# yonkshi/SPAIR_pytorch

Hardware: AMD Instinct MI355X
Metric: SPAIR train images/sec + ELBO, 128x128 scattered-MNIST, batch 256 (higher is better)
Workload: dtype bf16

## Files before the change

### include/spair_hip.h

```cpp
#pragma once
#include <stddef.h>
#include <stdint.h>
#ifdef __cplusplus
extern "C" {
#endif

#define SPAIR_DTYPE_F32 0
#define SPAIR_DTYPE_BF16 1

typedef struct SpairDims {
    int B, C, I, G;
    int P, A, F, NP;
    int n_conv;
    int conv_k[8], conv_s[8], conv_c[8];
    int pad_pre, pad_post, cell_px;
    int dtype;
    int align_corners;
    float anchor;
    float max_yx, min_yx, max_hw, min_hw;
    float obj_logit_scale, alpha_logit_scale, alpha_logit_bias;
    float vae_beta;
    float prior_mean[6], prior_std[6];
    int obj_conv, oc_n;
    int oc_k[4], oc_s[4], oc_c[4];
    int lookback;
    int Iw, Gw, pad_post_w;
} SpairDims;

#define SPAIR_ABI_VERSION 3
int spair_abi_version(void);

typedef struct SpairStep {
    float wheel;
    float count_prior_prob;
    float kl_scale;
    int train;
    int flags;
    int draw_noise;
    unsigned long long noise_seed;
    int* status;
    int* status_host;
} SpairStep;

int spair_init(void);

int spair_param_count(const SpairDims* d);
int spair_param_info(const SpairDims* d, int idx, char* name, int name_cap, int64_t* offset, int64_t* shape4, int* ndim);
int64_t spair_param_total(const SpairDims* d);
int64_t spair_workspace_bytes(const SpairDims* d);

typedef struct SpairStepIO {
    const float* params;
    const float* x;
    float* eps_box;
    float* eps_attr;
    float* eps_depth;
    float* u_pres;
    void* workspace;
    float* loss_out;
    float* recon;
    float* z_where;
    float* z_pres;
    float* inv_den;
    const float* grad_loss;
    float* grads;
    void* ev_decoder;
    void* ev_cells;
    void* ev_backbone;
    const float* grad_recon;
    const float* grad_z_where;
    const float* grad_z_pres;
    float* aux_scratch;
    float* grad_x;
    void* x_scratch;
    int bce_target;
} SpairStepIO;
int spair_forward(const SpairDims* d, const SpairStep* st, const SpairStepIO* io, void* stream);
int spair_backward(const SpairDims* d, const SpairStep* st, const SpairStepIO* io, void* stream);
int spair_grad_buckets(const SpairDims* d, int64_t* lo3, int64_t* hi3);
int64_t spair_input_grad_scratch_bytes(const SpairDims* d);
int spair_adam(float* params, const float* grads, float* exp_avg, float* exp_avg_sq, int64_t n, float lr,
               float beta1, float beta2, float eps, int step, void* stream);
int spair_adam_guarded(float* params, const float* grads, float* exp_avg, float* exp_avg_sq, int64_t n, float lr,
                       float beta1, float beta2, float eps, int step, const int* skip, int* counters, void* stream);
int spair_host_word_alloc(int** out);
int spair_host_word_free(int* word);
int spair_export_map(const SpairDims* d, const void* workspace, int which, float* out, void* stream);
int spair_chain_stamps(const SpairDims* d, const void* workspace, unsigned long long* out, int n, void* stream);
int spair_chain_stamp_layout(int* fwd_per_wavefront, int* fwd_glimpse_interval, int* bwd_per_wavefront);
#define SPAIR_STEP_PLAN_INTS 38
#define SPAIR_RENDER_MMA 0
#define SPAIR_RENDER_GEN2 1
#define SPAIR_RENDER_GEN1 2
#define SPAIR_RENDER_COLOUR 3
#define SPAIR_CONV_GEMM 0
#define SPAIR_CONV_PATCH 1
#define SPAIR_CONV_PER_CLASS 2
#define SPAIR_CONV_PW_STACK 3
#define SPAIR_STEM_PATCH 0
#define SPAIR_STEM_GEMM 1
#define SPAIR_STEM_WGRAD16 2
#define SPAIR_STEM_GENERIC 3
int spair_step_plan(const SpairDims* d, const void* workspace, int flags, int input_grad, int* out, int n);
int spair_workspace_view(const SpairDims* d, const void* workspace, int flags, int input_grad, const char* name, long long* out);
int spair_workspace_view_name(const SpairDims* d, int idx, char* name, int name_cap);
int spair_chain_stamp_wavefronts(const SpairDims* d);
int spair_chain_sync_status(const SpairDims* d, const void* workspace, int* out, void* stream);
int spair_noise_fill(const SpairDims* d, uint64_t seed, float* eps_box, float* eps_attr, float* eps_depth, float* u_pres, void* stream);

int spair_prof_enable(int enable);
int spair_prof_select(unsigned long long slot_mask);
int spair_prof_read(float* ms, int* counts, int nslots);

int spair_gemm_nt(const float* A, int lda, const void* B, int ldb, float* C, int ldc, int M, int N, int K,
                  const float* bias, const float* relu_mask, int ldmask, int relu, int accumulate, int dtype,
                  void* stream);
int spair_gemm_tn(const float* A, int lda, const float* B, int ldb, float* C, int ldc, int M, int N, int R,
                  int dtype, void* stream);
int spair_gemm_nt_conv(const float* In, const int* conv13, const void* B, int ldb, float* C, int ldc, int M,
                       int N, int K, const float* bias, const float* relu_mask, int ldmask, int relu,
                       int accumulate, const int* cmap8, int dtype, void* stream);
int spair_gemm_tn_conv(const float* A, int lda, const float* In, const int* conv13, float* C, int ldc, int M,
                       int N, int R, int dtype, void* stream);
int spair_colsum(const float* A, int lda, int R, int N, float* out, void* stream);
int spair_objconv_gather(int transposed, const float* in, const long long* in6, const float* W, const float* bias, float* out,
                         const long long* out6, const float* gate, int k, int s, int relu, long long R, void* stream);
int spair_objconv_wgrad(const float* small, const long long* small6, const float* big, const long long* big6, float* G,
                        float* bias_small, int k, int s, long long R, void* stream);
int spair_gemm_nt16(const void* A, int lda, const void* B, int ldb, void* C, int ldc, int M, int N, int K,
                    const float* bias, const void* relu_mask, int ldmask, int mask_bf16, int relu, int c_bf16,
                    const int* conv13, const int* cmap8, void* stream);
int spair_gemm_tn16(const void* A, int lda, const void* B, int ldb, int b_bf16, float* C, int ldc, int M, int N,
                    int R, const int* conv13, int cw_cin, int cw_taps, float* colsum_out, float* scratch,
                    long long scratch_floats, void* stream);
int spair_stem_wgrad16(const void* dY, const float* xpad, float* dW, float* db, float* scratch,
                       long long scratch_floats, int B, int Hin, int stride, int Hout, void* stream);
int spair_conv1x1_stack_fwd16(const void* X, const void* const* W, const int* ldw, const int* cout,
                              const float* const* bias, void* const* Y, float* Ylast, int ldlast, int M, int L,
                              void* stream);
int spair_conv1x1_stack_bwd16(const void* dY, int ldd, int kd, const void* const* Wd, const int* ldw, const int* cout,
                              const void* const* gate, void* const* dX, int M, int L, void* stream);
int spair_metrics(const float* z_where, const float* z_pres, const float* bbox, const float* count, int B, int G,
                  int image_side, int K, float* scratch, float* out, void* stream);
int spair_batch_jaccard(const float* box_a, const float* box_b, int B, int A, int Bn, float* iou, void* stream);
int spair_scenes_generate(uint64_t seed, long long first, int B, int I, int K, int size_min, int size_max, float* image,
                          float* bbox, long long* count, float* scratch, void* stream);
int spair_cast_bf16(const float* src, int ld_src, void* dst, int ld_dst, long long rows, int cols, void* stream);
int spair_stn_glimpse_fwd(const float* x, const float* nbox, int B, float* glimpse, int ld_gl, int R, int C,
                          int I, int P, int align_corners, void* stream);
int spair_stn_glimpse_bwd(const float* x, const float* nbox, int B, const float* dglimpse, int ld_gl,
                          float* dnbox, int R, int C, int I, int P, int align_corners, void* stream);
int spair_input_grad_glimpse(const float* nbox, int B, int ncell, const float* dglimpse, int ld_gl, float* out, int C, int I, int P,
                             int align_corners, void* stream);
int spair_input_grad_stem(const void* dact0, int dact_bf16, const float* w, int B, int C, int I, int pad_pre, int k, int s, int Hout,
                          int Cout, const float* add, float* grad_x, void* stream);
int spair_stn_inverse_fwd(const float* sprites, const float* nbox, float* out, int N, int C, int P, int I, int align_corners,
                          void* stream);
int spair_stn_inverse_bwd(const float* sprites, const float* nbox, const float* grad_out, float* dsprites, float* dnbox, int N,
                          int C, int P, int I, int align_corners, void* stream);
int spair_render_fwd(const float* sprites, int ld_s, const float* nbox, const float* pres, const float* depth,
                     const float* x, float* recon, float* aux , float* bce_partial,
                     int B, int HW, int C, int I, int P, int align_corners, void* stream);
int spair_render_bwd(const float* sprites, int ld_s, const float* nbox, const float* pres, const float* depth,
                     const float* aux, const float* grad_loss, float* dlogits, float* dnbox, float* dpres, float* ddepth,
                     int B, int HW, int C, int I, int P, int align_corners, float obj_scale, float alpha_scale, void* stream);
int spair_render_fwd_rgb(const float* sprites, int ld_s, const float* nbox, const float* pres, const float* depth, const float* x,
                         float* recon, float* aux, float* bce_partial, int B, int HW, int C, int I, int P, int align_corners, void* stream);
int spair_render_bwd_rgb(const float* sprites, int ld_s, const float* nbox, const float* pres, const float* depth, const float* aux,
                         const float* grad_loss, float* dlogits, float* dnbox, float* dpres, float* ddepth, int B, int HW, int C, int I,
                         int P, int align_corners, float obj_scale, float alpha_scale, void* stream);
int spair_stem_conv_fwd(const float* x, const float* w, const float* bias, void* out, int B, int I, int pad_pre, int Hin, int Hout,
                        int Cout, int stride, int out_bf16, void* stream);
int spair_conv_s2k4_fwd16(const void* in16, const void* wf16, const float* bias, void* out16, int B, int Hin, int Hout, void* stream);
int spair_conv_s2k4_dgrad16(const void* dout16, const void* wd0, const void* wd1, const void* wd2, const void* wd3, const void* gate16,
                            void* out16, int B, int Ho, void* stream);
int spair_stem_conv_fwd_mask(const float* x, const float* w, const float* bias, void* out, void* mask8, int B, int I, int pad_pre, int Hin,
                             int Hout, void* stream);
int spair_conv_s2k4_dgrad16_bits(const void* dout16, const void* wd0, const void* wd1, const void* wd2, const void* wd3,
                                 const void* gate_bits8, void* out16, int B, int Ho, void* stream);
int64_t spair_decoder_fwd16_scratch_bytes(int n_out);
int spair_decoder_fwd16(const void* z_attr16, int ld_za, const float* W0, const float* b0, const float* W1, const float* b1,
                        const float* W2, const float* b2, void* H1, void* H2, void* sprites, int ld_s, long long N, int A, int n_out,
                        float obj_scale, float alpha_scale, float alpha_bias, void* stream_buf, void* stream);
int spair_decoder_bwd16(const void* dlogits16, int ld_s, const void* W2t16, int ld2, const void* W1t16, const void* W0t16, const void* H2,
                        const void* H1, void* dH2, void* dH1, float* d_z_attr, int ld_dza, long long N, int A, int n_out, void* stream);
int spair_render_fwd16(const void* sprites_f16, int ld_s, const float* nbox, const float* pres, const float* depth,
                       const float* x, float* recon, float* aux, float* bce_partial, int B, int HW, int C, int I, int P,
                       int align_corners, void* stream);
int spair_render_bwd16(const void* sprites_f16, int ld_s, const float* nbox, const float* pres, const float* depth,
                       const float* aux, const float* grad_loss, void* dlogits_bf16, float* dnbox, float* dpres, float* ddepth,
                       int B, int HW, int C, int I, int P, int align_corners, float obj_scale, float alpha_scale, void* stream);
int spair_render_prep(const float* nbox, const float* pres, const float* depth, void* records, int B, int HW, int I, int P,
                      int align_corners, void* stream);
int spair_render_fwd16m(const void* sprites_f16, int ld_s, const void* records, const float* x, float* recon, float* aux,
                        float* bce_partial, int B, int HW, int C, int I, int P, int align_corners, void* stream);
int spair_render_bwd16r(const void* sprites_f16, int ld_s, const float* nbox, const float* pres, const float* depth, const void* records,
                        const float* aux, const float* grad_loss, void* dlogits_bf16, float* dnbox, float* dpres, float* ddepth,
                        int B, int HW, int C, int I, int P, int align_corners, float obj_scale, float alpha_scale, void* stream);
int spair_render_owner(const void* sprites, int ld_s, int s16, int ch, const float* nbox, const float* pres, const float* depth,
                       const int* cidx, float threshold, int* owner, float* owner_weight, float* coverage, int* area, int B, int HW, int I,
                       int Iw, int P, int align_corners, void* stream);
int spair_parse_owner(const SpairDims* d, const void* workspace, int flags, float threshold, int* owner, float* owner_weight,
                      float* coverage, int* area, void* stream);
int spair_cell_rows(const SpairDims* d, const void* workspace, int* out, void* stream);
#ifdef __cplusplus
}
#endif
```

### spair_pytorch_amd/_lib.py

```python
import ctypes
import os

import torch

_HERE = os.path.dirname(os.path.abspath(__file__))
LIB_PATH = os.environ.get("SPAIR_HIP_LIB") or os.path.join(_HERE, "libspair_hip.so")

_ERR = {-1: "bad shape", -2: "unsupported dtype", -3: "kernel launch failed", -4: "unsupported configuration",
        -5: "misaligned leading dimension / size"}

_lib = None
ABI_VERSION = 3


class SpairHipError(RuntimeError):
    pass


class SpairDims(ctypes.Structure):
    _fields_ = [("B", ctypes.c_int), ("C", ctypes.c_int), ("I", ctypes.c_int), ("G", ctypes.c_int),
                ("P", ctypes.c_int), ("A", ctypes.c_int), ("F", ctypes.c_int), ("NP", ctypes.c_int),
                ("n_conv", ctypes.c_int), ("conv_k", ctypes.c_int * 8), ("conv_s", ctypes.c_int * 8),
                ("conv_c", ctypes.c_int * 8), ("pad_pre", ctypes.c_int), ("pad_post", ctypes.c_int),
                ("cell_px", ctypes.c_int), ("dtype", ctypes.c_int), ("align_corners", ctypes.c_int),
                ("anchor", ctypes.c_float), ("max_yx", ctypes.c_float), ("min_yx", ctypes.c_float),
                ("max_hw", ctypes.c_float), ("min_hw", ctypes.c_float), ("obj_logit_scale", ctypes.c_float),
                ("alpha_logit_scale", ctypes.c_float), ("alpha_logit_bias", ctypes.c_float),
                ("vae_beta", ctypes.c_float), ("prior_mean", ctypes.c_float * 6), ("prior_std", ctypes.c_float * 6),
                ("obj_conv", ctypes.c_int), ("oc_n", ctypes.c_int), ("oc_k", ctypes.c_int * 4), ("oc_s", ctypes.c_int * 4),
                ("oc_c", ctypes.c_int * 4), ("lookback", ctypes.c_int),
                ("Iw", ctypes.c_int), ("Gw", ctypes.c_int), ("pad_post_w", ctypes.c_int)]


class SpairStep(ctypes.Structure):
    _fields_ = [("wheel", ctypes.c_float), ("count_prior_prob", ctypes.c_float), ("kl_scale", ctypes.c_float),
                ("train", ctypes.c_int), ("flags", ctypes.c_int), ("draw_noise", ctypes.c_int), ("noise_seed", ctypes.c_uint64),
                ("status", ctypes.c_void_p), ("status_host", ctypes.c_void_p)]


class SpairStepIO(ctypes.Structure):
    _fields_ = [(n, ctypes.c_void_p) for n in (
        "params", "x", "eps_box", "eps_attr", "eps_depth", "u_pres", "workspace",
        "loss_out", "recon", "z_where", "z_pres", "inv_den",
        "grad_loss", "grads", "ev_decoder", "ev_cells", "ev_backbone",
        "grad_recon", "grad_z_where", "grad_z_pres", "aux_scratch", "grad_x", "x_scratch")] + [("bce_target", ctypes.c_int)]


_STEP_ARGS = [ctypes.POINTER(SpairDims), ctypes.POINTER(SpairStep), ctypes.POINTER(SpairStepIO), ctypes.c_void_p]


def lib():
    global _lib
    if _lib is None:
        if not os.path.exists(LIB_PATH):
            raise SpairHipError(
                "libspair_hip.so is not built (%s). Run `python -c 'import __graft_entry__ as g; g.build()'` "
                "or `python -m spair_pytorch_amd._build`. There is no CPU/PyTorch fallback." % LIB_PATH)
        h = ctypes.CDLL(LIB_PATH)
        got = h.spair_abi_version() if hasattr(h, "spair_abi_version") else None
        if got != ABI_VERSION:
            raise SpairHipError("%s has ABI version %s, this package needs %d: rebuild it (python -m spair_pytorch_amd._build)"
                                % (LIB_PATH, got, ABI_VERSION))
        for f, args in ((h.spair_forward, _STEP_ARGS), (h.spair_backward, _STEP_ARGS),
                        (h.spair_step_plan, [ctypes.POINTER(SpairDims), ctypes.c_void_p, ctypes.c_int, ctypes.c_int,
                                             ctypes.POINTER(ctypes.c_int), ctypes.c_int])):
            f.argtypes, f.restype = args, ctypes.c_int
        _declare_parse(h)
        _lib = h
    return _lib


def _declare_parse(h):
    vp, i, f = ctypes.c_void_p, ctypes.c_int, ctypes.c_float
    h.spair_render_owner.argtypes = [vp, i, i, i, vp, vp, vp, vp, f, vp, vp, vp, vp, i, i, i, i, i, i, vp]
    h.spair_parse_owner.argtypes = [ctypes.POINTER(SpairDims), vp, i, f, vp, vp, vp, vp, vp]
    h.spair_cell_rows.argtypes = [ctypes.POINTER(SpairDims), vp, vp, vp]
    for fn in (h.spair_render_owner, h.spair_parse_owner, h.spair_cell_rows):
        fn.restype = i


def check(rc, what):
    if rc != 0:
        raise SpairHipError("%s failed: %s (code %d)" % (what, _ERR.get(rc, "unknown"), rc))


def ptr(t):
    if t is None:
        return ctypes.c_void_p(0)
    return ctypes.c_void_p(t.data_ptr())


def stream():
    return ctypes.c_void_p(torch.cuda.current_stream().cuda_stream)


RENDER_FAMILIES = ("MMA", "GEN2", "GEN1", "COLOUR")


def step_plan(dims, workspace, flags=0):
    out = (ctypes.c_int * 8)()
    check(lib().spair_step_plan(ctypes.byref(dims), int(workspace), int(flags), 0, out, 8), "spair_step_plan")
    return dict(fwd=RENDER_FAMILIES[out[0]], bwd=RENDER_FAMILIES[out[1]], rec=bool(out[2]), s16=bool(out[3]), g16=bool(out[4]),
                chain=bool(out[5]), dec_fused=bool(out[6]))


CONV_KERNELS = ("GEMM", "PATCH", "PER_CLASS", "PW_STACK")
STEM_WGRADS = ("PATCH", "GEMM", "WGRAD16", "GENERIC")
STEP_PLAN_INTS = 38


def step_plan_n(dims, workspace, flags=0, input_grad=False):
    out = (ctypes.c_int * STEP_PLAN_INTS)()
    check(lib().spair_step_plan(ctypes.byref(dims), int(workspace), int(flags), int(bool(input_grad)), out, STEP_PLAN_INTS),
          "spair_step_plan")
    layers = range(dims.n_conv)
    return dict(side=bool(out[8]), dec_dgrad_fused=bool(out[9]), dec_wgrad_grouped=bool(out[10]), dec_wgrad_late=bool(out[11]), pw0=out[12],
                stem=STEM_WGRADS[out[13]], fwd=tuple(CONV_KERNELS[out[14 + i]] for i in layers),
                dgrad=tuple(CONV_KERNELS[out[22 + i]] for i in layers), gate_bits=tuple(bool(out[30 + i]) for i in layers))


VIEW_DTYPES = (torch.float32, torch.bfloat16, torch.float16)


def workspace_view_names(dims):
    f, buf, names = lib().spair_workspace_view_name, ctypes.create_string_buffer(128), []
    while f(ctypes.byref(dims), len(names), buf, 128) == 0:
        names.append(buf.value.decode())
    return names


def workspace_view(dims, workspace, name, flags=0, input_grad=False):
    out = (ctypes.c_longlong * 6)()
    check(lib().spair_workspace_view(ctypes.byref(dims), ctypes.c_void_p(int(workspace)), int(flags), int(bool(input_grad)),
                                     name.encode(), out), "spair_workspace_view(%s)" % name)
    return dict(offset=out[0], rows=out[1], cols=out[2], ld=out[3], dtype=VIEW_DTYPES[out[4]], written=bool(out[5]))


def render_owner(sprites, channels, nbox, pres, depth, B, HW, I, Iw, P, align_corners=False, threshold=0.5, cell_rows=None):
    if sprites.dtype not in (torch.float16, torch.float32) or sprites.stride(1) != 1:
        raise SpairHipError("sprites must be fp16 or fp32 rows")
    dev = sprites.device
    owner = torch.empty(B, I, Iw, device=dev, dtype=torch.int32)
    weight, cover = (torch.empty(B, I, Iw, device=dev, dtype=torch.float32) for _ in range(2))
    area = torch.empty(B, HW, device=dev, dtype=torch.int32)
    nbox, pres, depth = (t.contiguous().float() for t in (nbox, pres, depth))
    rows = None if cell_rows is None else cell_rows.to(device=dev, dtype=torch.int32).contiguous()
    if sprites.shape[0] != B * HW or nbox.numel() != 4 * B * HW or pres.numel() != B * HW or depth.numel() != B * HW or \
            (rows is not None and rows.numel() != HW):
        raise SpairHipError("render_owner: operands do not have B * HW rows")
    check(lib().spair_render_owner(ptr(sprites), int(sprites.stride(0)), int(sprites.dtype == torch.float16), int(channels), ptr(nbox),
                                   ptr(pres), ptr(depth), ptr(rows), float(threshold), ptr(owner), ptr(weight), ptr(cover), ptr(area),
                                   int(B), int(HW), int(I), int(Iw), int(P), int(bool(align_corners)), stream()), "spair_render_owner")
    return owner, weight, cover, area
```

### spair_pytorch_amd/csrc/backbone.h

```cpp
#pragma once
#include "common.h"
#include "spair_hip.h"

bool conv_s2k4_patch_fwd16_supported(int B, int Hin, int Hout, int cin, int cout, int k, int s_);
int conv_s2k4_patch_fwd16(const void* in, const void* wf, const float* bias, void* out, int B, int Hin, int Hout, int cin, int cout, int k, int s_,
                          hipStream_t s, void* mask = nullptr);
bool conv_s2k4_patch_dgrad16_supported(int B, int Ho, int hin, int cin, int cout, int k, int s_);
bool conv_s2k4_patch_dgrad16_stem_supported(int B, int Ho, int hin, int cin, int cout, int k, int s_, int stem_hin, int stem_s, long long stem_part_cap);
int conv_s2k4_patch_dgrad16(const void* dout, const void* const* wd, const void* gate, void* out, int B, int Ho, int hin, int cin, int cout, int k,
                            int s_, const float* stem_xp, int stem_hin, int stem_s, float* stem_part, long long stem_part_cap, float* stem_dw,
                            float* stem_db, hipStream_t s, const void* gate_bits = nullptr);

enum ConvKernel { CONV_GEMM = SPAIR_CONV_GEMM, CONV_PATCH = SPAIR_CONV_PATCH, CONV_PER_CLASS = SPAIR_CONV_PER_CLASS, CONV_PW_STACK = SPAIR_CONV_PW_STACK };
enum StemWgrad { STEM_PATCH = SPAIR_STEM_PATCH, STEM_GEMM = SPAIR_STEM_GEMM, STEM_WGRAD16 = SPAIR_STEM_WGRAD16, STEM_GENERIC = SPAIR_STEM_GENERIC };
```

### spair_pytorch_amd/csrc/chain.hip

```cpp
#include <type_traits>
#include "cell_math.h"
#include "chain.h"
#include "stn_math.h"

namespace {

constexpr int MT = 16;
constexpr int F = 100, REC = 56, CTX = 224, A_ = 50, NP = 100, GLN = 784, PG = 28;
constexpr int CH_PAD = 16;
constexpr int KC = 352, LD_XC = KC + CH_PAD;
constexpr int KX = 160, LD_XT = KX + CH_PAD;
constexpr int KG = 800, LD_GL = KG + CH_PAD;
constexpr int LD_H = 256 + CH_PAD;
constexpr int LD_O = 112;
static_assert(CHAIN_PACK[CW_BOX0].ksplit == F + CTX && CHAIN_PACK[CW_BOX0].kpad0 == KC && CHAIN_PACK[CW_BOX0].KT * 32 == KC, "box0 pack");
static_assert(CHAIN_PACK[CW_Z0].ksplit == F + CTX && CHAIN_PACK[CW_Z0].kpad0 == KC && CHAIN_PACK[CW_Z0].KT * 32 == KC + KX, "z0 pack");
static_assert(CHAIN_PACK[CW_OBJ0].ksplit == F + CTX && CHAIN_PACK[CW_OBJ0].kpad0 == KC && CHAIN_PACK[CW_OBJ0].KT * 32 == KC + KX, "obj0 pack");
static_assert(CHAIN_PACK[CW_ENC0].ksplit == GLN && CHAIN_PACK[CW_ENC0].kpad0 == KG && CHAIN_PACK[CW_ENC0].KT * 32 == KG, "enc0 pack");

__device__ __forceinline__ void lds_barrier() {
    asm volatile("s_waitcnt lgkmcnt(0)" ::: "memory");
    __builtin_amdgcn_s_barrier();
    asm volatile("" ::: "memory");
}
// ... 58 lines not shown
__device__ __forceinline__ float ch_log(float x) { return 0.693147180559945f * __builtin_amdgcn_logf(x); }

template <int PIECES, int PB>
__device__ __forceinline__ void copy_rows8(const void* lds_, int lds_pitch, void* hbm_, unsigned hbm_pitch, const int* row_r, int r0, int nc, int lane) {
    constexpr int NI = (PIECES + 7) / 8;
    typedef unsigned int uv __attribute__((ext_vector_type(PB / 4)));
    const int row = r0 + (lane >> 3), p0 = lane & 7;
    const char* src = reinterpret_cast<const char*>(lds_) + row * lds_pitch + p0 * PB;
    char* dst = reinterpret_cast<char*>(hbm_) + ((unsigned)row_r[row] * hbm_pitch + (unsigned)(p0 * PB));
    uv v[NI];
#pragma unroll
    for (int i = 0; i < NI; ++i)
        if (8 * (i + 1) <= PIECES || p0 + 8 * i < PIECES) v[i] = *reinterpret_cast<const uv*>(src + i * 8 * PB);
    if (row < nc) {
#pragma unroll
        for (int i = 0; i < NI; ++i)
            if (8 * (i + 1) <= PIECES || p0 + 8 * i < PIECES) CH_GSTORE(reinterpret_cast<uv*>(dst + i * 8 * PB), v[i]);
    }
}
template <int PIECES, int PB>
__device__ __forceinline__ void copy_rows_w(const void* lds, int lds_pitch, void* hbm, size_t hbm_pitch, const int* row_r, int nc, int lane) {
    copy_rows8<PIECES, PB>(lds, lds_pitch, hbm, (unsigned)hbm_pitch, row_r, 0, nc, lane);
    if (nc > 8) copy_rows8<PIECES, PB>(lds, lds_pitch, hbm, (unsigned)hbm_pitch, row_r, 8, nc, lane);
}

template <int KT0, int KT1, int NT, int NT0 = 0>
__device__ __forceinline__ void wg_gemm_t(const __bf16* inA, int ldA, const __bf16* inB, int ldB, const uint4* __restrict__ Wp, WPipe& p,
                                          const float* bias_l, f32x4& acc, int wave, int lane) {
    constexpr int KT = KT0 + KT1;
    static_assert(KT <= 16, "all activation fragments of the stage are held in registers");
    const uint4* base = tile_base<KT, NT, NT0>(Wp, wave, lane);
    const int nt = min(NT0 + wave, NT - 1);
    const __bf16* pa = inA + (lane & 15) * ldA + (lane >> 4) * 8;
    const __bf16* pb = (KT1 > 0) ? inB + (lane & 15) * ldB + (lane >> 4) * 8 : pa;
    bf16x8 x[KT];
#pragma unroll
    for (int kt = 0; kt < KT; ++kt)
        x[kt] = *reinterpret_cast<const bf16x8*>((kt < KT0) ? pa + kt * 32 : pb + (kt - KT0) * 32);
    acc = *reinterpret_cast<const f32x4*>(bias_l + nt * 16 + (lane >> 4) * 4);
    __builtin_amdgcn_sched_barrier(0);
#pragma unroll
    for (int f = 0; f < KT; ++f) {
        acc = __builtin_amdgcn_mfma_f32_16x16x32_bf16(as_frag(p.q[f % RD]), x[f], acc, 0, 0, 0);
        if (f + RD < KT) p.q[f % RD] = base[(size_t)(f + RD) * 64];
    }
}

template <int KTOT, int KSKIP, int NT>
__device__ __forceinline__ void pipe_fill_k(const uint4* __restrict__ Wp, WPipe& p, int wave, int lane) {
    const uint4* base = tile_base<KTOT, NT, 0>(Wp, wave, lane) + (size_t)KSKIP * 64;
#pragma unroll
    for (int f = 0; f < KTOT - KSKIP; ++f) p.q[f] = base[f * 64];
}
template <int KTOT, int KSKIP>
__device__ __forceinline__ void wg_gemm_tk(const __bf16* inB, int ldB, WPipe& p, f32x4& acc, int lane) {
    constexpr int KT = KTOT - KSKIP;
    static_assert(KT <= RD, "the remaining fragments sit in the ring");
    const __bf16* pb = inB + (lane & 15) * ldB + (lane >> 4) * 8;
    bf16x8 x[KT];
#pragma unroll
    for (int kt = 0; kt < KT; ++kt) x[kt] = *reinterpret_cast<const bf16x8*>(pb + kt * 32);
    __builtin_amdgcn_sched_barrier(0);
#pragma unroll
    for (int f = 0; f < KT; ++f) acc = __builtin_amdgcn_mfma_f32_16x16x32_bf16(as_frag(p.q[f]), x[f], acc, 0, 0, 0);
}
template <int KTOT, int NT, int K0, int N>
__device__ __forceinline__ void early_fill(const uint4* __restrict__ Wa, const uint4* __restrict__ Wb, WPipe& p, int wave, int lane) {
    static_assert(2 * N <= RD, "two fragments per k-step");
    const uint4* ba = tile_base<KTOT, NT, 0>(Wa, wave, lane) + (size_t)K0 * 64;
    const uint4* bb = tile_base<KTOT, NT, 0>(Wb, wave, lane) + (size_t)K0 * 64;
#pragma unroll
    for (int j = 0; j < N; ++j) { p.q[2 * j] = ba[j * 64]; p.q[2 * j + 1] = bb[j * 64]; }
}
template <int N>
__device__ __forceinline__ void early_mfma(const bf16x8 (&x)[N], const WPipe& p, f32x4& accA, f32x4& accB) {
#pragma unroll
    for (int j = 0; j < N; ++j) {
        accA = __builtin_amdgcn_mfma_f32_16x16x32_bf16(as_frag(p.q[2 * j]), x[j], accA, 0, 0, 0);
        accB = __builtin_amdgcn_mfma_f32_16x16x32_bf16(as_frag(p.q[2 * j + 1]), x[j], accB, 0, 0, 0);
    }
}
__device__ __forceinline__ void buf_store8_nt(__amdgpu_buffer_rsrc_t r, unsigned byte_off, unsigned lo, unsigned hi) {
    __builtin_amdgcn_raw_buffer_store_b64(u32x2_t{lo, hi}, r, (int)byte_off, 0, 2);
}
__device__ __forceinline__ void buf_store16_nt(__amdgpu_buffer_rsrc_t r, unsigned byte_off, u32x4_t v) {
    __builtin_amdgcn_raw_buffer_store_b128(v, r, (int)byte_off, 0, 2);
}

template <int KT>
__device__ __forceinline__ void pipe_fill2(const uint4* __restrict__ Wp, WPipe& p, int wave, int lane) {
    const uint4* b0 = Wp + (size_t)wave * KT * 64 + lane;
    const uint4* b1 = Wp + (size_t)(wave + 8) * KT * 64 + lane;
#pragma unroll
    for (int s = 0; s < RD; ++s) p.q[s] = ((s & 1) ? b1 : b0)[(s >> 1) * 64];
}
template <int KT, int CH, int NRES>
__device__ __forceinline__ void wg_gemm_t2(const __bf16* in, int ld, const uint4* __restrict__ Wp, WPipe& p, const uint4 (&res)[2 * NRES + 1],
                                           const float* bias_l, f32x4& acc0, f32x4& acc1, int wave, int lane) {
    static_assert(KT % CH == 0 && RD % 2 == 0, "whole chunks; ring slots alternate between the two tiles");
    constexpr int NCH = KT / CH, AH = RD / 2;
    constexpr int KS = KT - NRES;
    const uint4* b0 = Wp + (size_t)wave * KT * 64 + lane;
    const uint4* b1 = Wp + (size_t)(wave + 8) * KT * 64 + lane;
    const __bf16* pa = in + (lane & 15) * ld + (lane >> 4) * 8;
    bf16x8 x[2][CH];
#pragma unroll
    for (int j = 0; j < CH; ++j) x[0][j] = *reinterpret_cast<const bf16x8*>(pa + j * 32);
    acc0 = *reinterpret_cast<const f32x4*>(bias_l + wave * 16 + (lane >> 4) * 4);
    acc1 = *reinterpret_cast<const f32x4*>(bias_l + (wave + 8) * 16 + (lane >> 4) * 4);
#pragma unroll
    for (int c = 0; c < NCH; ++c) {
        if (c + 1 < NCH) {
#pragma unroll
            for (int j = 0; j < CH; ++j) x[(c + 1) & 1][j] = *reinterpret_cast<const bf16x8*>(pa + ((c + 1) * CH + j) * 32);
        }
        __builtin_amdgcn_sched_barrier(0);
#pragma unroll
        for (int j = 0; j < CH; ++j) {
            const int f = c * CH + j;
            if (f < KS) {
                acc0 = __builtin_amdgcn_mfma_f32_16x16x32_bf16(as_frag(p.q[(2 * f) % RD]), x[c & 1][j], acc0, 0, 0, 0);
                if (f + AH < KS) p.q[(2 * f) % RD] = b0[(size_t)(f + AH) * 64];
                acc1 = __builtin_amdgcn_mfma_f32_16x16x32_bf16(as_frag(p.q[(2 * f + 1) % RD]), x[c & 1][j], acc1, 0, 0, 0);
                if (f + AH < KS) p.q[(2 * f + 1) % RD] = b1[(size_t)(f + AH) * 64];
            } else {
                acc0 = __builtin_amdgcn_mfma_f32_16x16x32_bf16(as_frag(res[2 * (f - KS)]), x[c & 1][j], acc0, 0, 0, 0);
                acc1 = __builtin_amdgcn_mfma_f32_16x16x32_bf16(as_frag(res[2 * (f - KS) + 1]), x[c & 1][j], acc1, 0, 0, 0);
            }
        }
    }
}

template <int KT, int NT>
__device__ __forceinline__ void pipe_fill_s(const uint4* __restrict__ Whi, const uint4* __restrict__ Wlo, WPipe& p, int wave, int lane) {
    const size_t o = (size_t)min(wave, NT - 1) * KT * 64 + lane;
#pragma unroll
    for (int s_ = 0; s_ < RD; ++s_)
        if ((s_ >> 1) < KT) p.q[s_] = ((s_ & 1) ? Wlo : Whi)[o + (s_ >> 1) * 64];
}
template <int KT, int NT, int CH>
__device__ __forceinline__ void wg_gemm_s(const __bf16* inHi, const __bf16* inLo, int ld, const uint4* __restrict__ Whi, const uint4* __restrict__ Wlo,
                                          WPipe& p, const float* bias_l, f32x4& acc, int wave, int lane) {
    constexpr int NCH = (KT + CH - 1) / CH, AH = RD / 2;
    const int nt = min(wave, NT - 1);
    const size_t o = (size_t)nt * KT * 64 + lane;
    const int eoff = (lane & 15) * ld + (lane >> 4) * 8;
    bf16x8 xh[2][CH], xl[2][CH];
#pragma unroll
    for (int j = 0; j < CH; ++j)
        if (j < KT) { xh[0][j] = *reinterpret_cast<const bf16x8*>(inHi + eoff + j * 32); xl[0][j] = *reinterpret_cast<const bf16x8*>(inLo + eoff + j * 32); }
    acc = *reinterpret_cast<const f32x4*>(bias_l + nt * 16 + (lane >> 4) * 4);
#pragma unroll
    for (int c = 0; c < NCH; ++c) {
        if (c + 1 < NCH) {
#pragma unroll
            for (int j = 0; j < CH; ++j)
                if ((c + 1) * CH + j < KT) {
                    xh[(c + 1) & 1][j] = *reinterpret_cast<const bf16x8*>(inHi + eoff + ((c + 1) * CH + j) * 32);
                    xl[(c + 1) & 1][j] = *reinterpret_cast<const bf16x8*>(inLo + eoff + ((c + 1) * CH + j) * 32);
                }
        }
        __builtin_amdgcn_sched_barrier(0);
#pragma unroll
        for (int j = 0; j < CH; ++j) {
            const int f = c * CH + j;
            if (f < KT) {
                const bf16x8 wh = as_frag(p.q[(2 * f) % RD]), wl = as_frag(p.q[(2 * f + 1) % RD]);
                acc = __builtin_amdgcn_mfma_f32_16x16x32_bf16(wl, xh[c & 1][j], acc, 0, 0, 0);
                acc = __builtin_amdgcn_mfma_f32_16x16x32_bf16(wh, xl[c & 1][j], acc, 0, 0, 0);
// ... 1226 lines not shown
```

### spair_pytorch_amd/csrc/common.h

```cpp
#pragma once
#include <hip/hip_runtime.h>
#include <stdint.h>
#include <atomic>

#define SPAIR_OK 0
#define SPAIR_ERR_SHAPE (-1)
#define SPAIR_ERR_DTYPE (-2)
#define SPAIR_ERR_LAUNCH (-3)
#define SPAIR_ERR_UNSUPPORTED (-4)
#define SPAIR_ERR_ALIGN (-5)

#define SPAIR_F32 0
#define SPAIR_BF16 1

#define SPAIR_CHECK_LAUNCH()                                   \
    do {                                                       \
        hipError_t e__ = hipGetLastError();                    \
        if (e__ != hipSuccess) return SPAIR_ERR_LAUNCH;        \
    } while (0)


static inline int spair_dyn_lds_once(const void* fn, int bytes, std::atomic<unsigned long long>& done) {
    int dev = 0;
    if (hipGetDevice(&dev) != hipSuccess) return SPAIR_ERR_LAUNCH;
// ... 6 lines not shown
}
static inline int spair_num_cus() {
    static std::atomic<int> cus[64];
    int dev = 0;
    if (hipGetDevice(&dev) != hipSuccess) return 256;
    int n = cus[dev & 63].load(std::memory_order_relaxed);
    if (n <= 0) {
        if (hipDeviceGetAttribute(&n, hipDeviceAttributeMultiprocessorCount, dev) != hipSuccess || n <= 0) n = 256;
        cus[dev & 63].store(n, std::memory_order_relaxed);
    }
    return n;
}

typedef float f32x4 __attribute__((ext_vector_type(4)));
typedef __bf16 bf16x8 __attribute__((ext_vector_type(8)));
typedef __bf16 bf16x4 __attribute__((ext_vector_type(4)));
typedef unsigned short u16;

static inline int ceil_div(int a, int b) { return (a + b - 1) / b; }
static inline int round_up(int a, int b) { return ceil_div(a, b) * b; }

struct ConvDesc {
    int Hin, Win, Cin;
    int Hout, Wout;
    int kh, kw;
    int sy, sx;
    int dky, dkx;
    int oy, ox;
};

struct RowMap {
    int Hout, Wout;
    int Hc, Wc;
    int osy, osx, ooy, oox;
};

__device__ __forceinline__ float sigmoidf_(float x) { return 1.0f / (1.0f + expf(-x)); }

template <int CTRL>
__device__ __forceinline__ float dpp_add_(float v) {
    return v + __builtin_bit_cast(float, __builtin_amdgcn_update_dpp(0, __builtin_bit_cast(int, v), CTRL, 0xf, 0xf, true));
}
__device__ __forceinline__ float wave_reduce_sum(float v) {
    v = dpp_add_<0xB1>(v);
    v = dpp_add_<0x4E>(v);
    v = dpp_add_<0x141>(v);
    v = dpp_add_<0x140>(v);
    const int i = __builtin_bit_cast(int, v);
    return (__builtin_bit_cast(float, __builtin_amdgcn_readlane(i, 0)) + __builtin_bit_cast(float, __builtin_amdgcn_readlane(i, 16))) +
           (__builtin_bit_cast(float, __builtin_amdgcn_readlane(i, 32)) + __builtin_bit_cast(float, __builtin_amdgcn_readlane(i, 48)));
}

#if defined(__HIPCC__)
__device__ __forceinline__ void wave_lds_fence() {
    __builtin_amdgcn_fence(__ATOMIC_RELEASE, "wavefront");
    __builtin_amdgcn_wave_barrier();
    __builtin_amdgcn_fence(__ATOMIC_ACQUIRE, "wavefront");
}
typedef unsigned int u32x4_t __attribute__((ext_vector_type(4)));
#define BUF_OOB 0xfffffff0u
__device__ __forceinline__ __amdgpu_buffer_rsrc_t buf_rsrc(const void* p) {
    const unsigned long long a = reinterpret_cast<unsigned long long>(p);
    const unsigned lo = __builtin_amdgcn_readfirstlane((unsigned)a), hi = __builtin_amdgcn_readfirstlane((unsigned)(a >> 32));
    void* q = reinterpret_cast<void*>(((unsigned long long)hi << 32) | lo);
    return __builtin_amdgcn_make_buffer_rsrc(q, (short)0, (int)0xffffff00u, 0x00020000);
}
__device__ __forceinline__ uint4 buf_load16(__amdgpu_buffer_rsrc_t r, unsigned byte_off) {
    const u32x4_t v = __builtin_amdgcn_raw_buffer_load_b128(r, (int)byte_off, 0, 0);
    return make_uint4(v.x, v.y, v.z, v.w);
}
typedef unsigned int u32x2_t __attribute__((ext_vector_type(2)));
__device__ __forceinline__ void buf_store2(__amdgpu_buffer_rsrc_t r, unsigned byte_off, unsigned short bits) {
    __builtin_amdgcn_raw_buffer_store_b16((short)bits, r, (int)byte_off, 0, 0);
}
__device__ __forceinline__ void buf_store4(__amdgpu_buffer_rsrc_t r, unsigned byte_off, unsigned bits) {
    __builtin_amdgcn_raw_buffer_store_b32((int)bits, r, (int)byte_off, 0, 0);
}
__device__ __forceinline__ void buf_store8(__amdgpu_buffer_rsrc_t r, unsigned byte_off, unsigned lo, unsigned hi) {
    __builtin_amdgcn_raw_buffer_store_b64(u32x2_t{lo, hi}, r, (int)byte_off, 0, 0);
}
__device__ __forceinline__ void buf_store16(__amdgpu_buffer_rsrc_t r, unsigned byte_off, uint4 v) {
    __builtin_amdgcn_raw_buffer_store_b128(u32x4_t{v.x, v.y, v.z, v.w}, r, (int)byte_off, 0, 0);
}
#endif

__device__ __forceinline__ float block_reduce_sum_256(float v, float* smem4) {
    v = wave_reduce_sum(v);
    const int w = threadIdx.x >> 6;
    __syncthreads();
    if ((threadIdx.x & 63) == 0) smem4[w] = v;
    __syncthreads();
    return smem4[0] + smem4[1] + smem4[2] + smem4[3];
}
```

### spair_pytorch_amd/csrc/conv_s2.hip

```cpp
#include <numeric>
#include "common.h"
#include "backbone.h"

namespace {

constexpr int CP_BM = 256, CP_C = 128;
constexpr int CP_PPX = 392;
constexpr int CP_PATCH_B = CP_PPX * 128;
constexpr int CP_BT_B = 128 * 128;
constexpr int CP_NPIECE_W = 5;
constexpr int CP_LDS = 3 * CP_BT_B + 2 * CP_PATCH_B + 1024;
constexpr int CP_LDC = CP_C + 16;

struct ConvPatchArgs {
    const u16* in; const u16* wf; const float* bias; u16* out;
    unsigned char* mask;
    int B, Hin, Hout, M, K;
    int tpi;
};

template <int W>
__device__ __forceinline__ void cp_wait() { asm volatile("s_waitcnt vmcnt(%0)" ::"n"(W) : "memory"); }

__global__ __launch_bounds__(768, 3) void k_conv_s2k4_patch(ConvPatchArgs a) {
    extern __shared__ __attribute__((aligned(16))) char cp_sm[];
    char* bt = cp_sm;
    char* patch = cp_sm + 3 * CP_BT_B;
    const int tid = threadIdx.x, lane = tid & 63, wave = __builtin_amdgcn_readfirstlane(tid >> 6);
    const int q = lane >> 4, r16 = lane & 15;
    const int Hout = a.Hout, Ws = Hout + 1, Hs = Hout + 1;
    int m0, mend;
    if (a.tpi) {
        const int img = blockIdx.x / a.tpi, HH = Hout * Hout;
        m0 = img * HH + (blockIdx.x - img * a.tpi) * CP_BM;
        mend = min(m0 + CP_BM, (img + 1) * HH);
    } else {
        m0 = blockIdx.x * CP_BM;
        mend = min(m0 + CP_BM, a.M);
    }
    const int mlast = mend - 1;
    const int g0 = m0 / Hout, g1 = mlast / Hout;
    const int L0 = (g0 + g0 / Hout) * Ws + (m0 - g0 * Hout);
    const int npx = (g1 + g1 / Hout + 1) * Ws + (mlast - g1 * Hout) + 1 - L0 + 1;

    const bool loader = wave >= 8;
    const int lw = wave & 3;
    const int wm = (wave >> 1) & 3, wn = wave & 1;
    const __amdgpu_buffer_rsrc_t rin = buf_rsrc(a.in), rwf = buf_rsrc(a.wf);
    auto glds = [&](__amdgpu_buffer_rsrc_t rs, unsigned byte_off, char* dst) {
        __builtin_amdgcn_raw_ptr_buffer_load_lds(rs, (__attribute__((address_space(3))) void*)dst, 16, (int)byte_off, 0, 0, 0);
    };
    auto issue_b = [&](int kt) {
        const bool live = kt < (a.K >> 6);
        char* dst = bt + (kt % 3) * CP_BT_B;
#pragma unroll
        for (int p = 0; p < 4; ++p) {
            const int piece = lw * 4 + p, n = piece * 8 + (lane >> 3), pos = lane & 7, c = pos ^ (n & 7);
            glds(rwf, live ? ((unsigned)n * (unsigned)a.K + (unsigned)kt * 64u + (unsigned)c * 8u) * 2u : BUF_OOB, dst + piece * 1024);
        }
    };
    auto issue_patch = [&](int st, int part) {
        const int cls = st >> 1, half = st & 1, py = cls >> 1, px = cls & 1;
        char* dst = patch + (st & 1) * CP_PATCH_B;
#pragma unroll
        for (int e = 0; e < CP_NPIECE_W; ++e) {
            const int piece = (part * 4 + lw) * CP_NPIECE_W + e;
            const int pp = piece * 8 + (lane >> 3), pos = lane & 7, c = pos ^ (pp & 7);
            const int pg = L0 + pp, E = pg / Ws, xx = pg - E * Ws;
            const int b = E / Hs, yy = E - b * Hs;
            const bool ok = st < 8 && pp < npx && b < a.B;
            const unsigned off = (((unsigned)(b * a.Hin + 2 * yy + py) * (unsigned)a.Hin + (unsigned)(2 * xx + px)) * CP_C + half * 64 + c * 8) * 2u;
            glds(rin, ok ? off : BUF_OOB, piece < CP_PPX / 8 ? dst + piece * 1024 : cp_sm + 3 * CP_BT_B + 2 * CP_PATCH_B);
        }
    };

    f32x4 acc[4][4];
#pragma unroll
    for (int i = 0; i < 4; ++i)
#pragma unroll
        for (int j = 0; j < 4; ++j) acc[i][j] = (f32x4){0.f, 0.f, 0.f, 0.f};

    if (loader) {
#pragma unroll
        for (int part = 0; part < 3; ++part) issue_patch(0, part);
        issue_b(0);
        issue_b(1);
        cp_wait<4>();
        for (int st = 0; st < 8; ++st) {
#pragma unroll
            for (int j4 = 0; j4 < 4; ++j4) {
                const int kt = st * 4 + j4;
                __builtin_amdgcn_s_barrier();
                asm volatile("" ::: "memory");
                if (j4 != 3) issue_patch(st + 1, j4);
                issue_b(kt + 2);
                if (j4 == 3) cp_wait<4>(); else cp_wait<4 + CP_NPIECE_W>();
            }
        }
        __builtin_amdgcn_s_barrier();
    } else {
        int pbase[4];
#pragma unroll
        for (int i = 0; i < 4; ++i) {
            const int m = min(m0 + wm * 64 + i * 16 + r16, mlast);
            const int g = m / Hout, x = m - g * Hout;
            pbase[i] = (g + g / Hout) * Ws + x - L0;
        }
        for (int st = 0; st < 8; ++st) {
            const char* pb = patch + (st & 1) * CP_PATCH_B;
#pragma unroll
            for (int j4 = 0; j4 < 4; ++j4) {
                const int kt = st * 4 + j4;
                __builtin_amdgcn_s_barrier();
                asm volatile("" ::: "memory");
                const char* bs = bt + (kt % 3) * CP_BT_B;
                const int tap = (j4 >> 1) * Ws + (j4 & 1);
#pragma unroll
                for (int ks = 0; ks < 2; ++ks) {
                    bf16x8 af[4], bfr[4];
                    const int c = ks * 4 + q;
#pragma unroll
                    for (int i = 0; i < 4; ++i) {
                        const int pp = pbase[i] + tap;
                        af[i] = *reinterpret_cast<const bf16x8*>(pb + pp * 128 + ((c ^ (pp & 7)) << 4));
                    }
#pragma unroll
                    for (int j = 0; j < 4; ++j) {
                        const int n = wn * 64 + j * 16 + r16;
                        bfr[j] = *reinterpret_cast<const bf16x8*>(bs + n * 128 + ((c ^ (n & 7)) << 4));
                    }
#pragma unroll
                    for (int i = 0; i < 4; ++i)
#pragma unroll
                        for (int j = 0; j < 4; ++j) acc[i][j] = __builtin_amdgcn_mfma_f32_16x16x32_bf16(af[i], bfr[j], acc[i][j], 0, 0, 0);
                }
            }
        }
        __builtin_amdgcn_s_barrier();
    }
    asm volatile("s_waitcnt vmcnt(0)" ::: "memory");
    __syncthreads();

    __bf16* cs = reinterpret_cast<__bf16*>(patch);
    if (!loader) {
#pragma unroll
        for (int j = 0; j < 4; ++j) {
            const int n = wn * 64 + j * 16 + r16;
            const float bv = a.bias[n];
#pragma unroll
            for (int i = 0; i < 4; ++i)
#pragma unroll
                for (int r = 0; r < 4; ++r) cs[(wm * 64 + i * 16 + q * 4 + r) * CP_LDC + n] = (__bf16)fmaxf(acc[i][j][r] + bv, 0.f);
        }
    }
    __syncthreads();
    const __amdgpu_buffer_rsrc_t rout = buf_rsrc(a.out);
    if (tid < 512) {
#pragma unroll
        for (int it = 0; it < CP_BM / 32; ++it) {
            const int row = it * 32 + (tid >> 4), ch = (tid & 15) * 8;
            const uint4 v = *reinterpret_cast<const uint4*>(cs + row * CP_LDC + ch);
            buf_store16(rout, (m0 + row) < mend ? ((unsigned)(m0 + row) * CP_C + ch) * 2u : BUF_OOB, v);
            if (a.mask) {
                auto nz2 = [](unsigned w) { return (unsigned)((int)(w << 16) > 0) | ((unsigned)((int)w >> 16 > 0) << 1); };
                const unsigned byte = nz2(v.x) | (nz2(v.y) << 2) | (nz2(v.z) << 4) | (nz2(v.w) << 6);
                if ((m0 + row) < mend) a.mask[(size_t)(m0 + row) * 16 + (tid & 15)] = (unsigned char)byte;
            }
        }
    }
}

}

static int cp_plan(int B, int Hin, int Hout, int cin, int cout, int k, int s_, int& tiles_out, int& tpi_out) {
    if (cin != CP_C || cout != CP_C || k != 4 || s_ != 2 || Hin != 2 * Hout + 2 || B <= 0 || Hout <= 0) return SPAIR_ERR_UNSUPPORTED;
    const long long M = (long long)B * Hout * Hout;
    if (M * CP_C >= (1ll << 31) || (long long)B * Hin * Hin * CP_C >= (1ll << 31)) return SPAIR_ERR_UNSUPPORTED;
    auto window = [&](long long m0, long long ml) {
        const long long g0 = m0 / Hout, g1 = ml / Hout;
        return (int)((g1 + g1 / Hout + 1) * (Hout + 1) + (ml - g1 * Hout) + 1 - ((g0 + g0 / Hout) * (Hout + 1) + (m0 - g0 * Hout)) + 1);
    };
    int tiles = (int)((M + CP_BM - 1) / CP_BM), tpi = 0, worst = 0;
    const long long period = (long long)Hout * Hout / std::gcd((long long)CP_BM, (long long)Hout * Hout);
    const bool walk = std::min<long long>(tiles, period) <= 65536;
    for (int t = 0; walk && t < tiles && t < period; ++t)
        worst = std::max(worst, window((long long)t * CP_BM, std::min<long long>((long long)(t + 1) * CP_BM, M) - 1));
    if (walk && tiles > period) worst = std::max(worst, window((long long)(tiles - 1) * CP_BM, M - 1));
    if (!walk || worst > CP_PPX) {
        const int HH = Hout * Hout;
        tpi = (HH + CP_BM - 1) / CP_BM;
        worst = 0;
        for (int t = 0; t < tpi; ++t) worst = std::max(worst, window((long long)t * CP_BM, std::min<long long>((long long)(t + 1) * CP_BM, HH) - 1));
        if (worst > CP_PPX) return SPAIR_ERR_UNSUPPORTED;
        tiles = B * tpi;
    }
    tiles_out = tiles; tpi_out = tpi;
    return SPAIR_OK;
}
bool conv_s2k4_patch_fwd16_supported(int B, int Hin, int Hout, int cin, int cout, int k, int s_) {
    int t, p;
    return cp_plan(B, Hin, Hout, cin, cout, k, s_, t, p) == SPAIR_OK;
}
int conv_s2k4_patch_fwd16(const void* in, const void* wf, const float* bias, void* out, int B, int Hin, int Hout, int cin, int cout, int k, int s_,
                          hipStream_t s, void* mask) {
    int tiles = 0, tpi = 0;
    { const int rc = cp_plan(B, Hin, Hout, cin, cout, k, s_, tiles, tpi); if (rc != SPAIR_OK) return rc; }
    const long long M = (long long)B * Hout * Hout;
    static std::atomic<unsigned long long> attr_done{0};
    if (spair_dyn_lds_once(reinterpret_cast<const void*>(&k_conv_s2k4_patch), CP_LDS, attr_done) != SPAIR_OK) return SPAIR_ERR_LAUNCH;
    ConvPatchArgs a;
    a.in = reinterpret_cast<const u16*>(in); a.wf = reinterpret_cast<const u16*>(wf); a.bias = bias; a.out = reinterpret_cast<u16*>(out);
    a.mask = reinterpret_cast<unsigned char*>(mask);
    a.B = B; a.Hin = Hin; a.Hout = Hout; a.M = (int)M; a.K = 16 * CP_C; a.tpi = tpi;
    hipLaunchKernelGGL(k_conv_s2k4_patch, dim3(tiles), dim3(768), CP_LDS, s, a);
    SPAIR_CHECK_LAUNCH();
    return SPAIR_OK;
}

extern "C" int spair_conv_s2k4_fwd16(const void* in16, const void* wf16, const float* bias, void* out16, int B, int Hin, int Hout, void* stream) {
    return conv_s2k4_patch_fwd16(in16, wf16, bias, out16, B, Hin, Hout, 128, 128, 4, 2, (hipStream_t)stream);
}
```

### spair_pytorch_amd/csrc/engine.hip

```cpp
#include <string.h>
#include <stdio.h>
#include <algorithm>
#include <mutex>
#include <vector>

#include "backbone.h"
#include "cells.h"
#include "gemm.h"
#include "misc.h"
#include "chain.h"
#include "dec_fused.h"
#include "objconv.h"
#include "render.h"

#define TRY(expr)                      \
    do {                               \
        int rc__ = (expr);             \
        if (rc__ != SPAIR_OK) return rc__; \
    } while (0)


#define SP_PROF_SLOTS 24
#define SP_PROF_POOL 8192
struct ProfState {
// ... 23 lines not shown
    int i; hipStream_t s;
    ProfScope(int slot, hipStream_t st) : i(prof_begin(slot, st)), s(st) {}
    ~ProfScope() { prof_end(i, s); }
};

extern "C" int spair_prof_enable(int enable) {
    std::lock_guard<std::mutex> lock(g_prof_mu);
    if (enable && g_prof.n_events == 0) {
        for (int i = 0; i < 2 * SP_PROF_POOL; ++i)
            if (hipEventCreate(&g_prof.ev[i]) != hipSuccess) return SPAIR_ERR_LAUNCH;
        g_prof.n_events = 2 * SP_PROF_POOL;
    }
    g_prof.enabled = enable ? 1 : 0;
    if (enable == 1) g_prof.used = 0;
    return SPAIR_OK;
}
extern "C" int spair_prof_select(unsigned long long mask) {
    std::lock_guard<std::mutex> lock(g_prof_mu);
    g_prof.mask = mask;
    return SPAIR_OK;
}
extern "C" int spair_prof_read(float* ms, int* counts, int nslots) {
    std::lock_guard<std::mutex> lock(g_prof_mu);
    for (int i = 0; i < g_prof.used; ++i) {
        float t = 0.f;
        if (hipEventSynchronize(g_prof.ev[2 * i + 1]) != hipSuccess) return SPAIR_ERR_LAUNCH;
        if (hipEventElapsedTime(&t, g_prof.ev[2 * i], g_prof.ev[2 * i + 1]) != hipSuccess) return SPAIR_ERR_LAUNCH;
        const int sl = g_prof.slot[i];
        if (sl >= 0 && sl < nslots) { ms[sl] += t; counts[sl] += 1; }
    }
    g_prof.used = 0;
    return SPAIR_OK;
}
enum { PS_PREP = 0, PS_BACKBONE_FWD, PS_CELLS_FWD, PS_DECODER_FWD, PS_COUNT_KL, PS_RENDER_FWD, PS_LOSS, PS_RENDER_BWD, PS_DECODER_BWD,
       PS_CELLS_BWD, PS_CELLS_WGRAD, PS_BACKBONE_BWD, PS_CONV1_FWD, PS_DEC2_FWD, PS_STN_FWD, PS_ADAM, PS_DEC2_WGRAD, PS_DEC2_DGRAD };

static int validate(const SpairDims& d) {
    if (d.B <= 0 || d.I <= 0 || d.G <= 0 || d.P <= 0 || d.A <= 0 || d.F <= 0 || d.NP <= 0) return SPAIR_ERR_SHAPE;
    if (d.Iw <= 0 || d.Gw <= 0 || d.pad_post_w < 0 || d.pad_post < 0 || d.pad_pre < 0) return SPAIR_ERR_SHAPE;
    if (d.C < 1 || d.C > 3) return SPAIR_ERR_UNSUPPORTED;
    if (d.C != 1 && d.obj_conv) return SPAIR_ERR_UNSUPPORTED;
    if (d.n_conv < 1 || d.n_conv > SP_MAX_CONV) return SPAIR_ERR_SHAPE;
    if (d.dtype != SPAIR_F32 && d.dtype != SPAIR_BF16) return SPAIR_ERR_DTYPE;
    if ((d.F & 3) || (d.NP & 3)) return SPAIR_ERR_ALIGN;
    int h = d.I + d.pad_pre + d.pad_post, wd = d.Iw + d.pad_pre + d.pad_post_w;
    for (int i = 0; i < d.n_conv; ++i) {
        if (d.conv_k[i] < 1 || d.conv_s[i] < 1 || (d.conv_c[i] & 7)) return SPAIR_ERR_SHAPE;
        if (i > 0 && d.conv_k[i] > 1 && (d.conv_k[i] % d.conv_s[i] != 0 || d.conv_s[i] > 2)) return SPAIR_ERR_UNSUPPORTED;
        if (i > 0 && d.conv_k[i] == 1 && d.conv_s[i] != 1) return SPAIR_ERR_UNSUPPORTED;
        h = (h - d.conv_k[i]) / d.conv_s[i] + 1;
        wd = (wd - d.conv_k[i]) / d.conv_s[i] + 1;
    }
    if (h != d.G || wd != d.Gw) return SPAIR_ERR_SHAPE;
    if ((long long)d.G * d.Gw + 1 > 1025) return SPAIR_ERR_UNSUPPORTED;
    if (d.A + 5 > 64) return SPAIR_ERR_UNSUPPORTED;
    if (d.lookback < 0 || d.lookback > 3) return SPAIR_ERR_UNSUPPORTED;
    if (d.lookback > 1 && std::max(d.G, d.Gw) > 32) return SPAIR_ERR_UNSUPPORTED;
    if (d.obj_conv) {
        if (d.oc_n < 1 || d.oc_n > 4) return SPAIR_ERR_SHAPE;
        int hh = d.P, ci = d.C;
        for (int i = 0; i < d.oc_n; ++i) {
            if (d.oc_k[i] < 1 || d.oc_s[i] < 1 || d.oc_c[i] < 1 || d.oc_k[i] > hh) return SPAIR_ERR_SHAPE;
            if ((long long)ci * d.oc_c[i] * d.oc_k[i] * d.oc_k[i] > 256 * 36 || d.oc_c[i] > 256) return SPAIR_ERR_UNSUPPORTED;
            const int ho = (hh - d.oc_k[i]) / d.oc_s[i] + 1;
            hh = ho; ci = d.oc_c[i];
        }
        if (((ci * hh * hh) & 7) || ((d.P * d.P * (d.C + 1)) & 7)) return SPAIR_ERR_ALIGN;
        if ((long long)(d.C + 1) * d.oc_c[0] * d.oc_k[0] * d.oc_k[0] > 256 * 36) return SPAIR_ERR_UNSUPPORTED;
    }
    return SPAIR_OK;
}

struct StepPlan {
    bool use_chain;
    bool use_dec_fused;
    RenderPlan rp;
    bool use_side;
    int pw0;
    ConvKernel conv_fwd[SP_MAX_CONV + 1], conv_dgrad[SP_MAX_CONV + 1];
    bool gate_bits[SP_MAX_CONV + 1];
    bool stem_bits;
    StemWgrad stem_wgrad;
    bool stem_unpadded;
    bool dec_dgrad_fused;
    bool dec_wgrad_grouped;
    bool dec_wgrad_late;
};

static RenderGeom render_geom(const SpairDims& d, const CellLayout& L, const CellBufs* b) {
    return {b ? b->nbox : nullptr, b ? b->rec + (L.REC - 1) : nullptr, b ? b->rec + (L.REC - 2) : nullptr, L.ld_rec, d.B, L.HW, d.I, d.P,
            d.align_corners, d.Iw};
}

static bool decoder_small_wgrad_grouped_supported(const ParamLayout& PL, const CellLayout& L) {
    const LinSpec &l1 = PL.lin[LIN_DEC1], &l0 = PL.lin[LIN_DEC0];
    return l1.in <= 128 && l0.in <= 128 && !(l1.out & 7) && !(l0.out & 7) && ceil_div(l1.out, 128) + ceil_div(l0.out, 128) <= SPAIR_TN_MAX_TILES &&
           std::min(round_up(l1.in, 8), SP_DEC_H1) >= l1.in && std::min(round_up(l0.in, 8), L.ld_rec) >= l0.in &&
           (long long)L.N * std::max(SP_DEC_H2, L.ld_rec) < (1ll << 31);
}

static StepPlan plan_step(const SpairDims& d, int flags, bool input_grad, const void* base) {
    const CellLayout L = make_cell_layout(d);
    const ParamLayout PL = make_param_layout(d);
    StepPlan p = {};
    const bool b16 = d.dtype == SPAIR_BF16;
    const bool square = spair_dims_square(d);
    const int per = d.P * d.P * (d.C + 1), ld_s = round_up(per, 8);
    p.use_chain = square && chain_fwd_supported(d) && !(flags & 1) && !d.obj_conv;
    const float* at = static_cast<const float*>(base);
    p.rp = render_plan(d, render_geom(d, L, nullptr), ld_s, at, at, at);
    p.use_dec_fused = p.rp.s16  && !(flags & 16) && PL.lin[LIN_DEC0].out == SP_DEC_H1 && PL.lin[LIN_DEC1].out == SP_DEC_H2 &&
                      dec_fused_supported(d.A, per, L.ld_rec, L.N, ld_s);
    p.use_side = !(flags & 4);
    const ConvSpec& c0 = PL.conv[0];
    const bool grey4 = square && c0.cin == 1 && c0.k == 4 && c0.cout == 128;
    const bool fuse_stem = b16 && grey4 && !(flags & 8) && !input_grad;
    const bool patch = square && b16 && !(flags & 32);
    p.stem_wgrad = b16 && grey4 ? STEM_WGRAD16 : STEM_GENERIC;
    p.stem_unpadded = square && misc_conv0_reads_unpadded(d.B, c0.hin, d.C, c0.k, c0.cout);
    p.stem_bits = square && misc_conv0_writes_mask(d.B, c0.hin, d.C, c0.k, c0.s, c0.cout, b16);
    const int n = PL.n_conv;
    p.pw0 = n;
    for (int i = n - 1; b16 && i >= 1; --i) {
        const ConvSpec& cs = PL.conv[i];
        if (cs.k != 1 || cs.s != 1 || cs.cin != 128 || (i == n - 1 ? cs.cout > 128 : cs.cout != 128) || n - i > 4 || PL.conv[i - 1].cout != 128) break;
        p.pw0 = i;
    }
    if (n - p.pw0 < 2) p.pw0 = n;
    bool bits = p.stem_bits;
    for (int i = 1; i < n; ++i) {
        const ConvSpec& cs = PL.conv[i];
        if (i >= p.pw0) { p.conv_fwd[i] = p.conv_dgrad[i] = CONV_PW_STACK; continue; }
        p.conv_fwd[i] = patch && conv_s2k4_patch_fwd16_supported(d.B, cs.hin, cs.hout, cs.cin, cs.cout, cs.k, cs.s) ? CONV_PATCH : CONV_GEMM;
        if (cs.k == 1) p.conv_dgrad[i] = CONV_GEMM;
        else if (patch && conv_s2k4_patch_dgrad16_supported(d.B, cs.hout, cs.hin, cs.cin, cs.cout, cs.k, cs.s)) {
            p.conv_dgrad[i] = CONV_PATCH;
            p.gate_bits[i] = bits;
            if (i == 1 && fuse_stem &&
                conv_s2k4_patch_dgrad16_stem_supported(d.B, cs.hout, cs.hin, cs.cin, cs.cout, cs.k, cs.s, c0.hin, c0.s, SPAIR_TN_PART_FLOATS))
                p.stem_wgrad = STEM_PATCH;
        } else if (b16 && cs.hin % cs.s == 0 && cs.win % cs.s == 0 && cs.s * cs.s <= 4) {
            p.conv_dgrad[i] = CONV_GEMM;
            const int M = d.B * ceil_div(cs.hin, cs.s) * ceil_div(cs.win, cs.s);
            if (i == 1 && fuse_stem && spair_nt16_stem_fusable(M, cs.cin, cs.s * cs.s, c0.hin, c0.s, SPAIR_TN_PART_FLOATS)) p.stem_wgrad = STEM_GEMM;
        } else p.conv_dgrad[i] = CONV_PER_CLASS;
        bits = p.conv_fwd[i] == CONV_PATCH;
    }
    const bool dec16 = b16 && !PL.oc_n;
    p.dec_dgrad_fused = dec16 && !(flags & 64) && dec_fused_bwd_supported(PL.lin[LIN_DEC0].in, per, L.N, ld_s, ld_s, L.ld_rec);
    p.dec_wgrad_grouped = dec16 && decoder_small_wgrad_grouped_supported(PL, L);
    p.dec_wgrad_late = dec16 && p.use_side && p.use_chain;
    return p;
}

struct Ws {
    int *cell_h, *cell_w, *cidx, *nbr, *cons, *diag_start;
    void* conv_wf[SP_MAX_CONV + 1];
    void* conv_wd[SP_MAX_CONV + 1][4];
    void* lin_wf[LIN_COUNT];
    void* lin_wt[LIN_COUNT];
    float *bias_boxh, *bias_zh;
    void* chain_w[CW_COUNT];
    void* chain_wlo[3];
    void* chain_wt[CW_COUNT];
    void* dec_stream;
    float* xpad;
    float *act[SP_MAX_CONV + 1], *dact[SP_MAX_CONV + 1];
    void* dLog16;
    unsigned char* act0_bits;
    unsigned char* act_bits[SP_MAX_CONV + 1];
    float *feat, *dfeat;
    CellBufs cb;
    float *Za, *Hd1, *Hd2, *S, *dLog, *dHd2, *dHd1;
    void *Za16, *dfeat16;
    float *tn_part, *tn_part2;
    float *aux, *bce_partial, *kl_partial, *klp, *gedge_part;
    void* rrec;
    float *oc_ea[4], *oc_dea[4];
    float *oc_dh, *oc_ddh;
    float *oc_da[4], *oc_dda[4];
    int* chain_sync;
    float *bnd_rec, *bnd_grad;
    unsigned long long* stamps;
    int ld_feat, ld_s;
    size_t total;
};

struct Carver {
    char* base;
    size_t off;
    template <class T> T* take(size_t n) {
        off = (off + 255) & ~(size_t)255;
        T* p = base ? reinterpret_cast<T*>(base + off) : nullptr;
        off += n * sizeof(T);
        return p;
    }
    void* take_bytes(size_t n) { return take<char>(n); }
};

static Ws carve(const SpairDims& d, void* base) {
    Ws w;
    memset(&w, 0, sizeof(w));
    const CellLayout L = make_cell_layout(d);
    const ParamLayout PL = make_param_layout(d);
    const StepPlan p = plan_step(d, 0, false, nullptr);
    Carver c{reinterpret_cast<char*>(base), 0};
    const size_t es = d.dtype == SPAIR_BF16 ? 2 : 4;
    const size_t N = (size_t)L.N;
    w.cell_h = c.take<int>(L.HW); w.cell_w = c.take<int>(L.HW); w.cidx = c.take<int>(L.HW);
    w.nbr = c.take<int>(L.NB * L.HW); w.cons = c.take<int>(L.NB * L.HW); w.diag_start = c.take<int>((L.LB + 1) * (L.G - 1) + L.Gw + 2);
    for (int i = 1; i < PL.n_conv; ++i) {
        const ConvSpec& cs = PL.conv[i];
        const size_t K = (size_t)cs.k * cs.k * cs.cin;
        w.conv_wf[i] = c.take_bytes((size_t)cs.cout * round_up((int)K, 8) * es);
        if (cs.k == 1) w.conv_wd[i][0] = c.take_bytes((size_t)cs.cin * round_up(cs.cout, 8) * es);
        else for (int q = 0; q < cs.s * cs.s; ++q) {
            const int T = cs.k / cs.s;
            w.conv_wd[i][q] = c.take_bytes((size_t)cs.cin * T * T * cs.cout * es);
        }
    }
    auto lin_alloc = [&](int id, int rows_total) {
        w.lin_wf[id] = c.take_bytes((size_t)rows_total * round_up(PL.lin[id].in, 8) * es);
        w.lin_wt[id] = c.take_bytes((size_t)PL.lin[id].in * round_up(rows_total, 8) * es);
    };
    for (int id = 0; id < LIN_COUNT; ++id) {
        if (id == LIN_BOXH0 || id == LIN_ZH0) continue;
        int rows = PL.lin[id].out;
        if (id == LIN_BOXH1) rows += PL.lin[LIN_BOXH0].out;
        if (id == LIN_ZH1) rows += PL.lin[LIN_ZH0].out;
        lin_alloc(id, rows);
// ... 221 lines not shown
    c.T = S * (G - 1) + Gw;
    c.dstart.assign(c.T + 1, 0);
    int n = 0;
    for (int t = 0; t < c.T; ++t) {
        c.dstart[t] = n;
        for (int h = 0; h < G; ++h) {
            const int w = t - S * h;
            if (w >= 0 && w < Gw) ++n;
        }
    }
    c.dstart[c.T] = n;
}

static int nt(Ctx& c, const float* A, int lda, const void* B, int ldb, float* C, int ldc, int M, int N, int K, const float* bias,
              const float* mask, int ldmask, int relu, const ConvDesc* conv = nullptr, const RowMap* cmap = nullptr) {
    GemmNT g;
    memset(&g, 0, sizeof(g));
    g.A = A; g.lda = lda; g.B = B; g.ldb = ldb; g.C = C; g.ldc = ldc; g.M = M; g.N = N; g.K = K;
    g.bias = bias; g.mask = mask; g.ldmask = ldmask; g.relu = relu;
    if (conv) g.conv = *conv;
    if (cmap) { g.cmap = *cmap; g.use_cmap = 1; }
    return spair_gemm_nt_impl(g, conv != nullptr, c.d.dtype, c.s);
}
static int tn(Ctx& c, const float* A, int lda, int M, const float* B, int ldb, int N, float* C, int ldc, int R, float* colsum = nullptr,
              const ConvDesc* conv = nullptr, int cw_cin = 0, int cw_taps = 0) {
    GemmTN g;
    memset(&g, 0, sizeof(g));
    g.A = A; g.lda = lda; g.B = B; g.ldb = ldb; g.C = C; g.ldc = ldc;
    g.M = round_up(M, 4); g.N = round_up(N, 4); g.Mstore = M; g.Nstore = N; g.R = R; g.colsum_out = colsum;
    g.cw_cin = cw_cin; g.cw_taps = cw_taps;
    if (conv) g.conv = *conv;
    return spair_gemm_tn_impl(g, conv != nullptr, c.d.dtype, c.s);
}
static bool conv_kperm(const Ctx& c, const ConvSpec& cs) {
    return c.d.dtype == SPAIR_BF16 && cs.k > 1 && cs.s > 1 && cs.k % cs.s == 0 && cs.cin % 64 == 0 && cs.k * cs.k * cs.cin / 64 <= 64;
}
static void fill_ktab(GemmNT& g, const ConvSpec& cs) {
    const int T = cs.k / cs.s, TT = T * T, nh = cs.cin / 64;
    g.n_ktab = cs.k * cs.k * nh;
    for (int blk = 0; blk < g.n_ktab; ++blk) {
        const int tq = blk % TT, rr = blk / TT, h = rr % nh, cls = rr / nh;
        const int ky = cls / cs.s + cs.s * (tq / T), kx = cls % cs.s + cs.s * (tq % T);
        g.ktab[blk] = ((unsigned)ky << 24) | ((unsigned)kx << 16) | (unsigned)(h * 64);
    }
}
static int nt16(Ctx& c, const void* A, int lda, const void* B, int ldb, void* C, int ldc, int c_bf16, int M, int N, int K, const float* bias,
                const void* mask, int ldmask, int relu, const ConvDesc* conv = nullptr, const RowMap* cmap = nullptr,
                const ConvSpec* fwd_cs = nullptr) {
    GemmNT g;
    memset(&g, 0, sizeof(g));
    g.A = reinterpret_cast<const float*>(A); g.lda = lda; g.B = B; g.ldb = ldb; g.C = reinterpret_cast<float*>(C); g.ldc = ldc; g.c_bf16 = c_bf16;
    g.M = M; g.N = N; g.K = K; g.bias = bias; g.mask = reinterpret_cast<const float*>(mask); g.ldmask = ldmask; g.mask_bf16 = 1; g.relu = relu;
    if (conv) g.conv = *conv;
    if (cmap) { g.cmap = *cmap; g.use_cmap = 1; }
    if (fwd_cs && conv_kperm(c, *fwd_cs)) fill_ktab(g, *fwd_cs);
    return spair_gemm_nt16_impl(g, conv != nullptr, c.s);
}
static int tn16(Ctx& c, const void* A, int lda, int M, const void* B, int ldb, int N, bool b_bf16, float* C, int ldc, int R, float* colsum,
                const ConvDesc* conv = nullptr, int cw_cin = 0, int cw_taps = 0) {
    GemmTN g;
    memset(&g, 0, sizeof(g));
    g.A = reinterpret_cast<const float*>(A); g.lda = lda; g.B = reinterpret_cast<const float*>(B); g.ldb = ldb; g.C = C; g.ldc = ldc;
    g.M = round_up(M, 8); g.N = round_up(N, b_bf16 ? 8 : 4); g.Mstore = M; g.Nstore = N; g.R = R; g.colsum_out = colsum;
    g.cw_cin = cw_cin; g.cw_taps = cw_taps;
    g.part = c.tn_part; g.part_cap = SPAIR_TN_PART_FLOATS;
    if (conv) g.conv = *conv;
    return spair_gemm_tn16_impl(g, conv != nullptr, b_bf16, c.s);
}
static const void* bptr(const void* base, size_t elem_off, int dtype) {
    return reinterpret_cast<const char*>(base) + elem_off * (dtype == SPAIR_BF16 ? 2 : 4);
}

static int prep_weights(Ctx& c, bool need_dgrad, int part) {
    std::vector<PrepEntry> es;
    const int bf = c.d.dtype == SPAIR_BF16;
    auto push = [&](const float* src, void* dst, int rows, int cols, int ld, int mode, int bf16, int cin = 0, int cout = 0, int k = 0,
                    int py = 0, int px = 0, int T = 0, int s = 0) {
        PrepEntry e;
        memset(&e, 0, sizeof(e));
        e.src = src; e.dst = dst; e.rows = rows; e.cols = cols; e.ld = ld; e.mode = mode; e.bf16 = bf16;
        e.cin = cin; e.cout = cout; e.k = k; e.py = py; e.px = px; e.T = T; e.s = s;
        es.push_back(e);
    };
    for (int i = 1; part == 0 && i < c.PL.n_conv; ++i) {
        const ConvSpec& cs = c.PL.conv[i];
        const float* w = c.params + cs.w;
        const int K = cs.k * cs.k * cs.cin;
        if (cs.k == 1) {
            push(w, c.w.conv_wf[i], cs.cout, cs.cin, round_up(K, 8), 0, bf);
            if (need_dgrad) push(w, c.w.conv_wd[i][0], cs.cin, cs.cout, round_up(cs.cout, 8), 1, bf);
        } else {
            const bool perm = conv_kperm(c, cs);
            push(w, c.w.conv_wf[i], cs.cout, K, round_up(K, 8), 2, bf, cs.cin, cs.cout, cs.k, 0, 0, perm ? cs.k / cs.s : 0, perm ? cs.s : 0);
            if (need_dgrad) {
                const int T = cs.k / cs.s;
                for (int py = 0; py < cs.s; ++py)
                    for (int px = 0; px < cs.s; ++px)
                        push(w, c.w.conv_wd[i][py * cs.s + px], cs.cin, T * T * cs.cout, T * T * cs.cout, 3, bf, cs.cin, cs.cout, cs.k, py, px, T, cs.s);
            }
        }
    }
    for (int id = 0; part == 1 && id < LIN_COUNT; ++id) {
        if (id == LIN_BOXH0 || id == LIN_ZH0) continue;
        const LinSpec& l = c.PL.lin[id];
        if (!l.in || !l.out) continue;
        const int ldf = round_up(l.in, 8);
        int head0 = -1;
        if (id == LIN_BOXH1) head0 = LIN_BOXH0;
        if (id == LIN_ZH1) head0 = LIN_ZH0;
        const int rows_total = l.out + (head0 >= 0 ? c.PL.lin[head0].out : 0);
        const int ldt = round_up(rows_total, 8);
        push(c.params + l.w, c.w.lin_wf[id], l.out, l.in, ldf, 0, bf);
        if (need_dgrad) push(c.params + l.w, c.w.lin_wt[id], l.in, l.out, ldt, 1, bf);
        if (head0 >= 0) {
            const LinSpec& h = c.PL.lin[head0];
            push(c.params + h.w, const_cast<void*>(bptr(c.w.lin_wf[id], (size_t)l.out * ldf, c.d.dtype)), h.out, h.in, ldf, 0, bf);
            if (need_dgrad) push(c.params + h.w, const_cast<void*>(bptr(c.w.lin_wt[id], (size_t)l.out, c.d.dtype)), h.in, h.out, ldt, 1, bf);
        }
    }
    if (part == 1 && c.use_chain) {
        auto pack = [&](void* const* dst, int cw, int mode, int bf16) {
            const ChainPack& k = CHAIN_PACK[cw];
            for (int head = 0; head < (k.lin_head >= 0 ? 2 : 1); ++head) {
                const LinSpec& l = c.PL.lin[head ? k.lin_head : k.lin];
                PrepEntry e;
                memset(&e, 0, sizeof(e));
                e.src = c.params + l.w; e.dst = dst[cw]; e.rows = l.out; e.cols = l.in; e.mode = mode; e.bf16 = bf16;
                e.KT = mode == 4 ? k.KT : k.KTt; e.n_off = head ? c.L.NP : 0;
                if (mode == 4) { e.ksplit = k.ksplit; e.kpad0 = k.kpad0; }
                es.push_back(e);
            }
        };
        for (int cw = 0; cw < 3; ++cw) pack(c.w.chain_wlo, cw, 4, 2);
        for (int cw = 0; cw < CW_COUNT; ++cw) pack(c.w.chain_w, cw, 4, 1);
        for (int cw = 0; need_dgrad && cw < CW_COUNT; ++cw)
            if (CHAIN_PACK[cw].ntt) pack(c.w.chain_wt, cw, 5, 1);
    }
    if (part == 1 && c.use_dec_fused)
        TRY(dec_fused_pack(c.params + c.PL.lin[LIN_DEC0].w, c.params + c.PL.lin[LIN_DEC1].w, c.params + c.PL.lin[LIN_DEC2].w, c.d.A,
                           c.d.P * c.d.P * (c.d.C + 1), c.d.obj_logit_scale, c.d.alpha_logit_scale, c.w.dec_stream, c.s));
    if (part == 1) {
        push(c.params + c.PL.lin[LIN_BOXH1].b, c.w.bias_boxh, 1, c.L.NP, c.L.NP + 8, 0, 0);
        push(c.params + c.PL.lin[LIN_BOXH0].b, c.w.bias_boxh + c.L.NP, 1, 8, 8, 0, 0);
        push(c.params + c.PL.lin[LIN_ZH1].b, c.w.bias_zh, 1, c.L.NP, c.L.NP + 8, 0, 0);
        push(c.params + c.PL.lin[LIN_ZH0].b, c.w.bias_zh + c.L.NP, 1, 2, 8, 0, 0);
    }
    for (size_t i = 0; i < es.size(); i += SP_MAX_PREP) {
        PrepTable T;
        T.n = (int)std::min((size_t)SP_MAX_PREP, es.size() - i);
        for (int j = 0; j < T.n; ++j) T.e[j] = es[i + j];
        TRY(misc_prep(T, c.s));
    }
    return SPAIR_OK;
}

static ConvDesc fwd_desc(const ConvSpec& cs) {
    ConvDesc cd;
    cd.Hin = cs.hin; cd.Win = cs.win; cd.Cin = cs.cin; cd.Hout = cs.hout; cd.Wout = cs.wout; cd.kh = cs.k; cd.kw = cs.k;
    cd.sy = cs.s; cd.sx = cs.s; cd.dky = 1; cd.dkx = 1; cd.oy = 0; cd.ox = 0;
    return cd;
}

static int dgrad_class(const ConvSpec& cs, int py, int px, ConvDesc& dd, RowMap& rm) {
    const int T = cs.k / cs.s;
    const int Hc = (cs.hin - py + cs.s - 1) / cs.s, Wc = (cs.win - px + cs.s - 1) / cs.s;
    dd.Hin = cs.hout; dd.Win = cs.wout; dd.Cin = cs.cout; dd.Hout = Hc; dd.Wout = Wc; dd.kh = T; dd.kw = T;
    dd.sy = 1; dd.sx = 1; dd.dky = -1; dd.dkx = -1; dd.oy = 0; dd.ox = 0;
    rm.Hout = Hc; rm.Wout = Wc; rm.Hc = cs.hin; rm.Wc = cs.win; rm.osy = cs.s; rm.osx = cs.s; rm.ooy = py; rm.oox = px;
    return Hc > 0 && Wc > 0 ? Hc * Wc : 0;
}
static GemmNT dgrad_classes16(const Ctx& c, int i) {
    const ConvSpec &cs = c.PL.conv[i], &c0 = c.PL.conv[0];
    const int T = cs.k / cs.s;
    GemmNT g;
    memset(&g, 0, sizeof(g));
    g.M = c.d.B * dgrad_class(cs, 0, 0, g.conv, g.cmap); g.use_cmap = 1; g.N = cs.cin; g.K = T * T * cs.cout;
    g.ldb = g.K; g.C = c.w.dact[i - 1]; g.ldc = cs.cin; g.c_bf16 = 1; g.mask = c.w.act[i - 1]; g.ldmask = cs.cin; g.mask_bf16 = 1;
    g.nz = cs.s * cs.s;
    for (int q = 0; q < g.nz; ++q) g.Bz[q] = c.w.conv_wd[i][q];
    g.B = g.Bz[0];
    if (i == 1) { g.stem_xp = c.w.xpad; g.stem_hin = c0.hin; g.stem_s = c0.s; g.stem_part = c.w.tn_part; g.stem_part_cap = SPAIR_TN_PART_FLOATS; }
    return g;
}

static int make_ctx(Ctx& c, const SpairDims* d, const SpairStep* st, const SpairStepIO* io, void* stream, bool input_grad = false) {
    if (!d || !st || !io || !io->params || !io->x || !io->eps_box || !io->eps_attr || !io->eps_depth || !io->u_pres || !io->workspace)
        return SPAIR_ERR_SHAPE;
    c.d = spair_dims_norm(*d); c.st = *st;
    TRY(validate(c.d));
    d = &c.d;
    c.L = make_cell_layout(*d);
    c.PL = make_param_layout(*d);
    c.w = carve(*d, io->workspace);
    c.params = io->params; c.x = io->x; c.s = (hipStream_t)stream; c.tn_part = c.w.tn_part;
    CellHyper& H = c.H;
    H.wheel = st->wheel; H.kl_scale = st->kl_scale * d->vae_beta; H.img = (float)d->I; H.anchor = d->anchor;
    H.cell_over_img = (float)((double)d->cell_px / (double)d->I);
    H.img_w = (float)d->Iw;
    H.cell_over_w = (float)((double)d->cell_px / (double)d->Iw);
    H.max_yx = d->max_yx; H.min_yx = d->min_yx; H.max_hw = d->max_hw; H.min_hw = d->min_hw;
    H.range_yx = d->max_yx - d->min_yx; H.range_hw = d->max_hw - d->min_hw;
    for (int i = 0; i < 6; ++i) { H.prior_mean[i] = d->prior_mean[i]; H.prior_std[i] = d->prior_std[i]; }
    H.count_prior_prob = st->count_prior_prob;
    c.w.cb.edge = c.params + c.PL.edge;
    c.w.cb.eps_box = io->eps_box; c.w.cb.eps_attr = io->eps_attr; c.w.cb.eps_depth = io->eps_depth; c.w.cb.u_pres = io->u_pres;
    fill_diag(c);
    static_cast<StepPlan&>(c) = plan_step(*d, st->flags, input_grad, io->workspace);
    c.rg = render_geom(*d, c.L, &c.w.cb);
    return SPAIR_OK;
}

static int backbone_stem_fwd(Ctx& c) {
    const SpairDims& d = c.d;
    const int b16 = d.dtype == SPAIR_BF16;
    const ConvSpec& c0 = c.PL.conv[0];
    if (!c.stem_unpadded) TRY(misc_pad_input(c.x, c.w.xpad, d.B, d.C, d.I, d.Iw, d.pad_pre, c0.hin, c0.win, c.s));
    return misc_conv0_fwd(c.x, c.w.xpad, c.params + c0.w, c.params + c0.b, c.w.act[0], d.B, d.I, d.pad_pre, c0.hin, d.C, c0.k, c0.s, c0.hout,
                          c0.cout, b16, c.s, c.w.act0_bits, c0.win, c0.wout, c.stem_unpadded);
}
static int backbone_fwd(Ctx& c) {
    const SpairDims& d = c.d;
    const int b16 = d.dtype == SPAIR_BF16;
    const int pw0 = c.pw0;
    for (int i = 1; i < c.PL.n_conv; ++i) {
        const ConvSpec& cs = c.PL.conv[i];
        const bool last = (i == c.PL.n_conv - 1);
        const int M = d.B * cs.hout * cs.wout, K = cs.k * cs.k * cs.cin;
        if (c.conv_fwd[i] == CONV_PW_STACK) {
            const void* W[4]; const float* bias[4]; void* Y[4]; int ldw[4], cout[4];
            const int Lp = c.PL.n_conv - pw0;
            for (int l = 0; l < Lp; ++l) {
                const ConvSpec& q = c.PL.conv[pw0 + l];
                W[l] = c.w.conv_wf[pw0 + l]; ldw[l] = round_up(q.cin, 8); cout[l] = q.cout; bias[l] = c.params + q.b; Y[l] = c.w.act[pw0 + l];
            }
            TRY(spair_pw_stack_fwd16(c.w.act[pw0 - 1], W, ldw, cout, bias, Y, c.w.feat, c.w.ld_feat, M, Lp, c.s));
            break;
        }
        float* out = last ? c.w.feat : c.w.act[i];
        const int ldc = last ? c.w.ld_feat : cs.cout;
        const ConvDesc cd = fwd_desc(cs);
        if (c.conv_fwd[i] == CONV_PATCH) {
            ProfScope ps(i == 1 ? PS_CONV1_FWD : -1, c.s);
            TRY(conv_s2k4_patch_fwd16(c.w.act[i - 1], c.w.conv_wf[i], c.params + cs.b, out, d.B, cs.hin, cs.hout, cs.cin, cs.cout, cs.k, cs.s, c.s,
                                      c.w.act_bits[i]));
        } else if (b16) {
            ProfScope ps(i == 1 ? PS_CONV1_FWD : -1, c.s);
            TRY(nt16(c, c.w.act[i - 1], cs.cin, c.w.conv_wf[i], round_up(K, 8), out, ldc, last ? 0 : 1, M, cs.cout, round_up(K, 8),
                     c.params + cs.b, nullptr, 0, last ? 0 : 1, cs.k == 1 ? nullptr : &cd, nullptr, cs.k == 1 ? nullptr : &cs));
        } else if (cs.k == 1) {
            TRY(nt(c, c.w.act[i - 1], cs.cin, c.w.conv_wf[i], round_up(K, 8), out, ldc, M, cs.cout, round_up(K, 8), c.params + cs.b, nullptr, 0, last ? 0 : 1));
        } else {
            ProfScope ps(i == 1 ? PS_CONV1_FWD : -1, c.s);
            TRY(nt(c, c.w.act[i - 1], 0, c.w.conv_wf[i], round_up(K, 8), out, ldc, M, cs.cout, K, c.params + cs.b, nullptr, 0, last ? 0 : 1, &cd));
        }
    }
    return SPAIR_OK;
}

static int backbone_bwd16(Ctx& c, float* grads) {
    const SpairDims& d = c.d;
    const int last = c.PL.n_conv - 1, pw0 = c.pw0;
    const ConvSpec& c0 = c.PL.conv[0];
    const int N = d.B * d.G * d.Gw;
    if (!c.use_chain) TRY(spair_to_bf16(c.w.dfeat, c.w.ld_feat, c.w.dfeat16, c.w.ld_feat, N, c.w.ld_feat, c.s));
    if (pw0 <= last) {
        const void* Wd[4]; const void* gate[4]; void* dX[4]; int ldw[4], cout[4];
        const int Lp = last - pw0 + 1;
        for (int l = 0; l < Lp; ++l) {
            const int i = last - l;
            const ConvSpec& q = c.PL.conv[i];
            Wd[l] = c.w.conv_wd[i][0]; ldw[l] = round_up(q.cout, 8); cout[l] = q.cout; gate[l] = c.w.act[i - 1]; dX[l] = c.w.dact[i - 1];
        }
        TRY(spair_pw_stack_bwd16(c.w.dfeat16, c.w.ld_feat, c.PL.conv[last].cout, Wd, ldw, cout, gate, dX, N, Lp, c.s));
        GemmTN g;
        memset(&g, 0, sizeof(g));
        g.ngroup = last - pw0 + 1;
        for (int q = 0; q < g.ngroup; ++q) {
            const int i = pw0 + q;
            const ConvSpec& cs = c.PL.conv[i];
            GemmTN::Tile& t = g.tile[q];
            t.A = (i == last) ? c.w.dfeat16 : (const void*)c.w.dact[i];
            t.lda = (i == last) ? c.w.ld_feat : cs.cout;
            t.B = c.w.act[i - 1]; t.ldb = cs.cin;
            t.C = grads + cs.w; t.ldc = cs.cin; t.colsum = grads + cs.b;
            t.M = round_up(cs.cout, 8); t.N = cs.cin; t.Mstore = cs.cout; t.Nstore = cs.cin;
        }
        g.R = N;
        g.part = c.tn_part; g.part_cap = SPAIR_TN_PART_FLOATS;
        TRY(spair_gemm_tn16_impl(g, false, true, c.s));
    }
    for (int i = pw0 - 1; i >= 1; --i) {
        const ConvSpec& cs = c.PL.conv[i];
        const int M = d.B * cs.hout * cs.wout;
        const void* dout = (i == last) ? c.w.dfeat16 : (const void*)c.w.dact[i];
        const int ldd = (i == last) ? c.w.ld_feat : cs.cout;
        const void* in = c.w.act[i - 1];
        if (cs.k == 1) {
            TRY(tn16(c, dout, ldd, cs.cout, in, cs.cin, cs.cin, true, grads + cs.w, cs.cin, M, grads + cs.b));
            const int Kd = round_up(cs.cout, 8);
            TRY(nt16(c, dout, ldd, c.w.conv_wd[i][0], Kd, c.w.dact[i - 1], cs.cin, 1, M, cs.cin, Kd, nullptr, in, cs.cin, 0));
            continue;
        }
        const int K = cs.k * cs.k * cs.cin;
        const ConvDesc cd = fwd_desc(cs);
        TRY(tn16(c, dout, ldd, cs.cout, in, 0, K, true, grads + cs.w, K, M, grads + cs.b, &cd, cs.cin, cs.k * cs.k));
        const int T = cs.k / cs.s;
        if (c.conv_dgrad[i] == CONV_PATCH) {
            const bool stem = i == 1 && c.stem_wgrad == STEM_PATCH;
            const void* wd4[4] = {c.w.conv_wd[i][0], c.w.conv_wd[i][1], c.w.conv_wd[i][2], c.w.conv_wd[i][3]};
            TRY(conv_s2k4_patch_dgrad16(dout, wd4, in, c.w.dact[i - 1], d.B, cs.hout, cs.hin, cs.cin, cs.cout, cs.k, cs.s, stem ? c.w.xpad : nullptr,
                                        c0.hin, c0.s, stem ? c.w.tn_part : nullptr, SPAIR_TN_PART_FLOATS, grads + c0.w, grads + c0.b, c.s,
                                        !c.gate_bits[i] ? nullptr : i == 1 ? c.w.act0_bits : c.w.act_bits[i - 1]));
        } else if (c.conv_dgrad[i] == CONV_GEMM) {
            GemmNT g = dgrad_classes16(c, i);
            g.A = reinterpret_cast<const float*>(dout);
            if (i == 1) {
                g.stem_dw = grads + c0.w; g.stem_db = grads + c0.b;
                if (c.stem_wgrad != STEM_GEMM) g.stem_part = nullptr;
            }
            TRY(spair_gemm_nt16_impl(g, true, c.s));
        } else {
            for (int py = 0; py < cs.s; ++py)
                for (int px = 0; px < cs.s; ++px) {
                    ConvDesc dd; RowMap rm;
// ... 148 lines not shown
        const OcTensor in = oc_dec_act(c, i - 1, false);
        TRY(oc_layer_wgrad(c, in, dout, grads + t.w, nullptr, t.k, t.s, L.N));
        TRY(spair_colsum_impl(dout.p, t.cout, L.N * t.hout * t.hout, t.cout, grads + t.b, c.s));
        TRY(oc_gather(false, dout, c.params + t.w, nullptr, oc_dec_act(c, i - 1, true), i ? in : OcTensor{}, t.k, t.s, 0, L.N, c.s));
    }
    TRY(wgrad_lin(c, LIN_DEC0, c.w.oc_ddh, flat, c.w.Za, L.ld_rec, grads, L.N));
    return bwd_lin(c, LIN_DEC0, flat, c.w.oc_ddh, flat, P.g_attr_r, L.ld_rec, 0, L.N, nullptr, 0);
}

static int cells_fwd(Ctx& c) {
    const CellLayout& L = c.L;
    CellBufs& P = c.w.cb;
    const ParamLayout& PL = c.PL;
    const float* pr = c.params;
    if (c.use_chain) {
        ChainArgs a;
        a.L = L; a.P = P; a.H = c.H;
        for (int i = 0; i < CW_COUNT; ++i) a.w[i] = reinterpret_cast<const uint4*>(c.w.chain_w[i]);
        for (int i = 0; i < 3; ++i) a.wlo[i] = reinterpret_cast<const uint4*>(c.w.chain_wlo[i]);
        a.bias[CW_BOX0] = pr + PL.lin[LIN_BOX0].b; a.bias[CW_BOX1] = pr + PL.lin[LIN_BOX1].b; a.bias[CW_BOXH] = c.w.bias_boxh;
        a.bias[CW_ENC0] = pr + PL.lin[LIN_ENC0].b; a.bias[CW_ENC1] = pr + PL.lin[LIN_ENC1].b; a.bias[CW_ENC2] = pr + PL.lin[LIN_ENC2].b;
        a.bias[CW_Z0] = pr + PL.lin[LIN_Z0].b; a.bias[CW_Z1] = pr + PL.lin[LIN_Z1].b; a.bias[CW_ZH] = c.w.bias_zh;
        a.bias[CW_OBJ0] = pr + PL.lin[LIN_OBJ0].b; a.bias[CW_OBJ1] = pr + PL.lin[LIN_OBJ1].b; a.bias[CW_OBJ2] = pr + PL.lin[LIN_OBJ2].b;
        a.x = c.x; a.I = c.d.I; a.Pp = c.d.P; a.ac = c.d.align_corners;
        a.w_obj2 = pr + PL.lin[LIN_OBJ2].w; a.gedge = nullptr; a.stamps = (c.st.flags & 2) ? c.w.stamps : nullptr;
        a.nbands = chain_bands(c.d); a.sync = c.w.chain_sync; a.bnd_rec = c.w.bnd_rec; a.bnd_grad = c.w.bnd_grad;
        for (int i = 0; i < CW_COUNT; ++i) a.wt[i] = nullptr;
        return chain_fwd(a, c.s);
    }
    for (int t = 0; t < c.T; ++t) {
        const int r0 = c.dstart[t] * L.B, R = (c.dstart[t + 1] - c.dstart[t]) * L.B;
        TRY(cells_ctx_gather(L, P, r0, R, c.s));
        if (c.d.dtype == SPAIR_BF16 && (PL.lin[LIN_BOX0].in & 3) == 0) {
            TRY(fwd_lin_f32(c, LIN_BOX0, P.Xb, L.ld_xb, P.Hb1, SP_LDH, 0, r0, R, 1));
            TRY(fwd_lin_f32(c, LIN_BOX1, P.Hb1, SP_LDH, P.Hb2, SP_LDH, 0, r0, R, 1));
            TRY(fwd_lin_f32(c, LIN_BOXH1, P.Hb2, SP_LDH, P.Ob, L.ld_ob, 0, r0, R, 0));
            TRY(fwd_lin_f32(c, LIN_BOXH0, P.Hb2, SP_LDH, P.Ob, L.ld_ob, L.ob_lat, r0, R, 0));
        } else {
        TRY(fwd_lin(c, LIN_BOX0, P.Xb, L.ld_xb, P.Hb1, SP_LDH, r0, R, pr + PL.lin[LIN_BOX0].b, SP_H, 1));
        TRY(fwd_lin(c, LIN_BOX1, P.Hb1, SP_LDH, P.Hb2, SP_LDH, r0, R, pr + PL.lin[LIN_BOX1].b, SP_H, 1));
        TRY(fwd_lin(c, LIN_BOXH1, P.Hb2, SP_LDH, P.Ob, L.ld_ob, r0, R, c.w.bias_boxh, L.NP + 8, 0));
        }
        TRY(cells_box_sample(L, P, c.H, r0, R, c.s));
        { ProfScope ps(PS_STN_FWD, c.s); TRY(stn_glimpse_fwd(c.x, P.nbox, L.B, P.glimpse, L.ld_gl, r0, R, c.d.C, c.d.I, c.d.Iw, c.d.P, c.d.align_corners, chain_image_fp16(c.d),
                                                                c.s)); }
        if (PL.oc_n) TRY(oc_encoder_fwd(c, r0, R));
        else {
        TRY(fwd_lin(c, LIN_ENC0, P.glimpse, L.ld_gl, P.He1, SP_ENC_H1, r0, R, pr + PL.lin[LIN_ENC0].b, SP_ENC_H1, 1));
        TRY(fwd_lin(c, LIN_ENC1, P.He1, SP_ENC_H1, P.He2, SP_ENC_H2, r0, R, pr + PL.lin[LIN_ENC1].b, SP_ENC_H2, 1));
        TRY(fwd_lin(c, LIN_ENC2, P.He2, SP_ENC_H2, P.Oe, L.ld_oe, r0, R, pr + PL.lin[LIN_ENC2].b, 2 * L.A, 0));
        }
        TRY(cells_attr_sample(L, P, r0, R, c.s));
        TRY(fwd_lin(c, LIN_Z0, P.Xz, L.ld_x, P.Hz1, SP_LDH, r0, R, pr + PL.lin[LIN_Z0].b, SP_H, 1));
        TRY(fwd_lin(c, LIN_Z1, P.Hz1, SP_LDH, P.Hz2, SP_LDH, r0, R, pr + PL.lin[LIN_Z1].b, SP_H, 1));
        TRY(fwd_lin(c, LIN_ZH1, P.Hz2, SP_LDH, P.Oz, L.ld_oz, r0, R, c.w.bias_zh, L.NP + 2, 0));
        TRY(cells_depth_sample(L, P, c.H, r0, R, c.s));
        TRY(fwd_lin(c, LIN_OBJ0, P.Xo, L.ld_x, P.Ho1, SP_LDH, r0, R, pr + PL.lin[LIN_OBJ0].b, SP_H, 1));
        TRY(fwd_lin(c, LIN_OBJ1, P.Ho1, SP_LDH, P.Ho2, SP_LDH, r0, R, pr + PL.lin[LIN_OBJ1].b, SP_H, 1));
        TRY(fwd_lin(c, LIN_OBJ2, P.Ho2, SP_LDH, P.Oo, L.ld_oo, r0, R, pr + PL.lin[LIN_OBJ2].b, 1, 0));
        TRY(cells_pres_sample(L, P, c.H, r0, R, c.s));
    }
    return SPAIR_OK;
}

extern "C" int spair_forward(const SpairDims* d, const SpairStep* st, const SpairStepIO* io, void* stream) {
    Ctx c;
    TRY(make_ctx(c, d, st, io, stream));
    d = &c.d;
    if (!io->loss_out || !io->recon || !io->z_where || !io->z_pres) return SPAIR_ERR_SHAPE;
    const CellLayout& L = c.L;
    CellBufs& P = c.w.cb;
    P.z_where = io->z_where; P.z_pres = io->z_pres;
    SideStream* side = nullptr;
    if (c.use_side) TRY(side_stream(side));
    std::unique_lock<std::mutex> enq_lock;
    if (side) enq_lock = std::unique_lock<std::mutex>(side->enq_mu);
    {
        if (side) TRY(stream_link(c.s, side->s, side->ev[2]));
        OnHelper on_helper(c, side);
        {
            ProfScope ps(PS_PREP, c.s);
            TRY(prep_weights(c, st->train != 0, 0));
            if (side && hipEventRecord(side->ev[3], side->s) != hipSuccess) return SPAIR_ERR_LAUNCH;
            TRY(cells_init_tables(d->G, d->Gw, c.L.LB, c.w.cell_h, c.w.cell_w, c.w.cidx, c.w.nbr, c.w.cons, c.w.diag_start, c.s));
            if (st->draw_noise)
                TRY(spair_noise_fill(d, st->noise_seed, io->eps_box, io->eps_attr, io->eps_depth, io->u_pres, c.s));
            TRY(prep_weights(c, st->train != 0, 1));
        }
        if (side && hipEventRecord(side->ev[4], side->s) != hipSuccess) return SPAIR_ERR_LAUNCH;
        if (c.stem_unpadded) TRY(misc_pad_input(c.x, c.w.xpad, d->B, d->C, d->I, d->Iw, d->pad_pre, c.PL.conv[0].hin, c.PL.conv[0].win, c.s));
    }
    const int ps_bb = prof_begin(PS_BACKBONE_FWD, c.s);
    TRY(backbone_stem_fwd(c));
    if (side && hipStreamWaitEvent(c.s, side->ev[3], 0) != hipSuccess) return SPAIR_ERR_LAUNCH;
    TRY(backbone_fwd(c));
    prof_end(ps_bb, c.s);
    if (side && hipStreamWaitEvent(c.s, side->ev[4], 0) != hipSuccess) return SPAIR_ERR_LAUNCH;
    { ProfScope ps(PS_CELLS_FWD, c.s); TRY(cells_fwd(c)); }
    {
        hipStream_t ks = side ? side->s : c.s;
        if (side) TRY(stream_link(c.s, ks, side->ev[0]));
        { ProfScope ps(PS_COUNT_KL, ks); TRY(loss_count_kl(L, P, st->count_prior_prob, c.w.klp, ks)); }
        const bool gauss_on_main = side && d->G > 16;
        if (!gauss_on_main) TRY(loss_gauss_kl(L, P, c.H, c.w.kl_partial, ks));
        if (side && hipEventRecord(side->ev[1], ks) != hipSuccess) return SPAIR_ERR_LAUNCH;
        if (gauss_on_main) TRY(loss_gauss_kl(L, P, c.H, c.w.kl_partial, c.s));
    }
    if (c.rp.rec) TRY(render_prep(c.rg, c.w.rrec, c.s));
    const ParamLayout& PL = c.PL;
    const int N = L.N;
    const int per = d->P * d->P * (d->C + 1);
    {
        ProfScope ps(PS_DECODER_FWD, c.s);
        const int b16 = d->dtype == SPAIR_BF16;
        const int K0 = round_up(PL.lin[LIN_DEC0].in, 8), K2 = round_up(PL.lin[LIN_DEC2].in, 8);
        if (b16 && !c.use_chain) TRY(spair_to_bf16(c.w.Za, L.ld_rec, c.w.Za16, L.ld_rec, N, L.ld_rec, c.s));
        if (PL.oc_n) {
            TRY(oc_decoder_fwd(c));
        } else if (c.use_dec_fused) {
            ProfScope p2(PS_DEC2_FWD, c.s);
            TRY(dec_fused_fwd(c.w.Za16, L.ld_rec, c.w.dec_stream, c.params + PL.lin[LIN_DEC0].b, c.params + PL.lin[LIN_DEC1].b, c.params + PL.lin[LIN_DEC2].b,
                              c.w.Hd1, c.w.Hd2, c.w.S, c.w.ld_s, N, d->A, per, d->obj_logit_scale, d->alpha_logit_scale, d->alpha_logit_bias, c.s));
        } else {
        if (b16) {
            TRY(nt16(c, c.w.Za16, L.ld_rec, c.w.lin_wf[LIN_DEC0], K0, c.w.Hd1, SP_DEC_H1, 1, N, SP_DEC_H1, K0, c.params + PL.lin[LIN_DEC0].b, nullptr, 0, 1));
            TRY(nt16(c, c.w.Hd1, SP_DEC_H1, c.w.lin_wf[LIN_DEC1], SP_DEC_H1, c.w.Hd2, SP_DEC_H2, 1, N, SP_DEC_H2, SP_DEC_H1,
                     c.params + PL.lin[LIN_DEC1].b, nullptr, 0, 1));
        } else {
            TRY(fwd_lin(c, LIN_DEC0, c.w.Za, L.ld_rec, c.w.Hd1, SP_DEC_H1, 0, N, c.params + PL.lin[LIN_DEC0].b, SP_DEC_H1, 1));
            TRY(fwd_lin(c, LIN_DEC1, c.w.Hd1, SP_DEC_H1, c.w.Hd2, SP_DEC_H2, 0, N, c.params + PL.lin[LIN_DEC1].b, SP_DEC_H2, 1));
        }
        {
            ProfScope p2(PS_DEC2_FWD, c.s);
            GemmNT g;
            memset(&g, 0, sizeof(g));
            g.A = c.w.Hd2; g.lda = SP_DEC_H2; g.B = c.w.lin_wf[LIN_DEC2]; g.ldb = K2; g.C = c.w.S; g.ldc = c.w.ld_s; g.M = N; g.N = per; g.K = K2;
            g.bias = c.params + PL.lin[LIN_DEC2].b; g.sprite_ch = d->C + 1;
            g.c_bf16 = c.rp.s16;
            g.obj_scale = d->obj_logit_scale; g.alpha_scale = d->alpha_logit_scale; g.alpha_bias = d->alpha_logit_bias;
            if (b16) TRY(spair_gemm_nt16_impl(g, false, c.s));
            else TRY(spair_gemm_nt_impl(g, false, d->dtype, c.s));
        }
        }
    }
    {
        ProfScope ps(PS_RENDER_FWD, c.s);
        float* const aux = st->train ? c.w.aux : nullptr;
        if (c.rp.fwd == RENDER_MMA) TRY(render_fwd_mma(c.rg, c.w.S, c.w.ld_s, c.w.rrec, c.x, io->recon, aux, c.w.bce_partial, io->inv_den, c.s));
        else if (c.rp.fwd == RENDER_GEN2) TRY(render_fwd2(c.rg, c.w.S, c.w.ld_s, c.rp.s16, c.x, io->recon, aux, c.w.bce_partial, io->inv_den, c.s));
        else if (c.rp.fwd == RENDER_GEN1) TRY(render_fwd1(c.rg, c.w.S, c.w.ld_s, c.rp.s16, c.x, io->recon, aux, c.w.bce_partial, io->inv_den, c.s));
        else TRY(render_fwd_c(c.rg, c.w.S, c.w.ld_s, d->C, c.x, io->recon, aux, c.w.bce_partial, io->inv_den, c.s));
    }
    if (side && hipStreamWaitEvent(c.s, side->ev[1], 0) != hipSuccess) return SPAIR_ERR_LAUNCH;
    ProfScope psl(PS_LOSS, c.s);
    TRY(loss_finalize(c.w.bce_partial, render_num_blocks(d->B, d->I, d->Iw), c.w.kl_partial, loss_gauss_kl_blocks(L), c.w.klp, d->B,
                      st->kl_scale, d->vae_beta, io->loss_out,
                      c.use_chain && c.w.chain_sync ? c.w.chain_sync + CHAIN_SYNC_STICKY(d->B, chain_bands(*d)) : nullptr, st->status,
                      st->status_host, c.s));
    return SPAIR_OK;
}

static int bwd_lin(Ctx& c, int id, int out_total, const float* dOut, int ldo, float* dX, int ldx, int r0, int R, const float* mask, int ldmask) {
    const int K = round_up(out_total, 8);
    return nt(c, dOut + (size_t)r0 * ldo, ldo, c.w.lin_wt[id], K, dX + (size_t)r0 * ldx, ldx, R, c.PL.lin[id].in, K, nullptr,
              mask ? mask + (size_t)r0 * ldmask : nullptr, ldmask, 0);
}
static int wgrad_lin(Ctx& c, int id, const float* dOut, int ldo, const float* In, int ldi, float* grads, int R) {
    const LinSpec& l = c.PL.lin[id];
    return tn(c, dOut, ldo, l.out, In, ldi, l.in, grads + l.w, l.in, R, grads + l.b);
}

static int cells_wgrad_grouped(Ctx& c, float* grads) {
    const CellLayout& L = c.L;
    const CellBufs& P = c.w.cb;
    GemmTN g;
    memset(&g, 0, sizeof(g));
    int nt = 0;
    bool fits = true;
// ... 223 lines not shown
        TRY(cells_bwd_box(L, P, c.H, r0, R, c.s));
        TRY(bwd_lin(c, LIN_BOXH1, L.NP + 8, P.dOb, L.ld_ob, P.dHb2, SP_LDH, r0, R, P.Hb2, SP_LDH));
        TRY(bwd_lin(c, LIN_BOX1, SP_H, P.dHb2, SP_LDH, P.dHb1, SP_LDH, r0, R, P.Hb1, SP_LDH));
        TRY(bwd_lin(c, LIN_BOX0, SP_H, P.dHb1, SP_LDH, P.dXb, L.ld_xb, r0, R, nullptr, 0));
    }
    TRY(cells_dfeat_edge(L, P, grads + PL.edge, c.s));
    }
    prof_end(ps_cells, c.s);
    {
        if (side) TRY(stream_link(c.s, side->s, side->ev[2]));
        OnHelper on_helper(c, side);
        if (c.dec_wgrad_late) TRY(decoder_wgrads16(c, grads, io->ev_decoder));
        const int ps_wg = prof_begin(PS_CELLS_WGRAD, c.s);
        if (c.use_chain) {
            TRY(cells_wgrad_grouped(c, grads));
            TRY(chain_edge_reduce(chain_args, c.s));
        } else {
        TRY(wgrad_lin(c, LIN_BOX0, P.dHb1, SP_LDH, P.Xb, L.ld_xb, grads, N));
        TRY(wgrad_lin(c, LIN_BOX1, P.dHb2, SP_LDH, P.Hb1, SP_LDH, grads, N));
        TRY(wgrad_lin(c, LIN_BOXH1, P.dOb, L.ld_ob, P.Hb2, SP_LDH, grads, N));
        TRY(wgrad_lin(c, LIN_BOXH0, P.dOb + L.ob_lat, L.ld_ob, P.Hb2, SP_LDH, grads, N));
        if (PL.oc_n) TRY(oc_encoder_wgrad(c, grads));
        else {
        TRY(wgrad_lin(c, LIN_ENC0, P.dHe1, SP_ENC_H1, P.glimpse, L.ld_gl, grads, N));
        TRY(wgrad_lin(c, LIN_ENC1, P.dHe2, SP_ENC_H2, P.He1, SP_ENC_H1, grads, N));
        TRY(wgrad_lin(c, LIN_ENC2, P.dOe, L.ld_oe, P.He2, SP_ENC_H2, grads, N));
        }
        TRY(wgrad_lin(c, LIN_Z0, P.dHz1, SP_LDH, P.Xz, L.ld_x, grads, N));
        TRY(wgrad_lin(c, LIN_Z1, P.dHz2, SP_LDH, P.Hz1, SP_LDH, grads, N));
        TRY(wgrad_lin(c, LIN_ZH1, P.dOz, L.ld_oz, P.Hz2, SP_LDH, grads, N));
        TRY(wgrad_lin(c, LIN_ZH0, P.dOz + L.oz_lat, L.ld_oz, P.Hz2, SP_LDH, grads, N));
        TRY(wgrad_lin(c, LIN_OBJ0, P.dHo1, SP_LDH, P.Xo, L.ld_x, grads, N));
        TRY(wgrad_lin(c, LIN_OBJ1, P.dHo2, SP_LDH, P.Ho1, SP_LDH, grads, N));
        TRY(wgrad_lin(c, LIN_OBJ2, P.dOo, L.ld_oo, P.Ho2, SP_LDH, grads, N));
        }
        prof_end(ps_wg, c.s);
        TRY(record_ready(io->ev_cells, c.s));
        if (side && hipEventRecord(side->ev[3], side->s) != hipSuccess) return SPAIR_ERR_LAUNCH;
    }
    { ProfScope ps(PS_BACKBONE_BWD, c.s); TRY(backbone_bwd(c, grads)); }
    if (side && hipStreamWaitEvent(c.s, side->ev[3], 0) != hipSuccess) return SPAIR_ERR_LAUNCH;
    TRY(record_ready(io->ev_backbone, c.s));
    if (io->grad_x) {
        if (c.use_chain) {
            const LinSpec& e0 = PL.lin[LIN_ENC0];
            const int K = round_up(e0.out, 8);
            TRY(nt16(c, P.dHe1, SP_ENC_H1, c.w.lin_wt[LIN_ENC0], K, P.dGl, L.ld_gl, 0, N, e0.in, K, nullptr, nullptr, 0, 0));
        }
        float* const x_scratch = static_cast<float*>(io->x_scratch);
        TRY(input_grad_glimpse(P.nbox, d->B, d->G * d->Gw, P.dGl, L.ld_gl, x_scratch, d->C, d->I, d->Iw, d->P, d->align_corners, c.s));
        const ConvSpec& c0 = PL.conv[0];
        TRY(input_grad_stem(c.w.dact[0], b16, c.params + c0.w, d->B, d->C, d->I, d->Iw, d->pad_pre, c0.k, c0.s, c0.hout, c0.wout, c0.cout, x_scratch,
                            c.w.aux,
                            io->bce_target ? grad_loss : nullptr, io->grad_x, c.s));
    }
    return SPAIR_OK;
}

extern "C" int spair_chain_stamps(const SpairDims* d0, const void* workspace, unsigned long long* out, int n, void* stream) {
    if (!d0 || !workspace || !out || n > 4096) return SPAIR_ERR_SHAPE;
    const SpairDims dn = spair_dims_norm(*d0), *d = &dn;
    TRY(validate(*d));
    const Ws w = carve(*d, const_cast<void*>(workspace));
    if (hipMemcpyAsync(out, w.stamps, sizeof(unsigned long long) * n, hipMemcpyDeviceToDevice, (hipStream_t)stream) != hipSuccess) return SPAIR_ERR_LAUNCH;
    return SPAIR_OK;
}

static_assert(SPAIR_RENDER_MMA == RENDER_MMA && SPAIR_RENDER_GEN2 == RENDER_GEN2 && SPAIR_RENDER_GEN1 == RENDER_GEN1 &&
              SPAIR_RENDER_COLOUR == RENDER_COLOUR, "include/spair_hip.h names the RenderFamily values");
static_assert(SPAIR_STEP_PLAN_INTS == 14 + 3 * SP_MAX_CONV, "include/spair_hip.h lays out spair_step_plan");
extern "C" int spair_step_plan(const SpairDims* d0, const void* workspace, int flags, int input_grad, int* out, int n) {
    if (!d0 || !workspace || !out) return SPAIR_ERR_SHAPE;
    const SpairDims dn = spair_dims_norm(*d0), *d = &dn;
    TRY(validate(*d));
    const StepPlan p = plan_step(*d, flags, input_grad != 0, workspace);
    int v[SPAIR_STEP_PLAN_INTS] = {p.rp.fwd, p.rp.bwd, p.rp.rec, p.rp.s16, p.rp.g16, p.use_chain, p.use_dec_fused, 0,
                                   p.use_side, p.dec_dgrad_fused, p.dec_wgrad_grouped, p.dec_wgrad_late, p.pw0, p.stem_wgrad};
    for (int i = 1; i <= SP_MAX_CONV; ++i) {
        const bool on = i <= d->n_conv;
        v[13 + i] = on ? p.conv_fwd[i] : -1; v[21 + i] = on ? p.conv_dgrad[i] : -1; v[29 + i] = on ? p.gate_bits[i] : -1;
    }
    for (int i = 0; i < std::min(n, SPAIR_STEP_PLAN_INTS); ++i) out[i] = v[i];
    return SPAIR_OK;
}

struct WsItem { char name[96]; const void* p; long long rows, cols, ld; int type, written; };

static const char* lin_param_name(const ParamLayout& PL, int id) {
    static const char* mlp[LIN_COUNT] = {"box_network.body.dense0", "box_network.body.dense1", "box_network.output_layers.0",
                                         "box_network.output_layers.1", "object_encoder.dense0", "object_encoder.dense1", "object_encoder.out",
                                         "z_network.body.dense0", "z_network.body.dense1", "z_network.output_layers.0", "z_network.output_layers.1",
                                         "obj_network.dense0", "obj_network.dense1", "obj_network.out", "object_decoder.dense0",
                                         "object_decoder.dense1", "object_decoder.out"};
    if (PL.oc_n && id == LIN_DEC0) return "object_decoder.inp";
    return mlp[id];
}

static std::vector<WsItem> ws_items(const SpairDims& d, const void* base, int flags, bool input_grad) {
    const Ws w = carve(d, const_cast<void*>(base));
    const StepPlan p = plan_step(d, flags, input_grad, base);
    const CellLayout L = make_cell_layout(d);
    const ParamLayout PL = make_param_layout(d);
    const CellBufs& b = w.cb;
    const bool b16 = d.dtype == SPAIR_BF16, oc = PL.oc_n > 0, chain = p.use_chain;
    const int et = b16 ? 1 : 0;
    const long long N = L.N;
    std::vector<WsItem> v;
    auto add = [&](const char* name, const void* ptr, long long rows, long long cols, long long ld, int type, bool written) {
        WsItem it;
        snprintf(it.name, sizeof(it.name), "%s", name);
        it.p = ptr; it.rows = rows; it.cols = cols; it.ld = ld; it.type = type; it.written = written ? 1 : 0;
        v.push_back(it);
    };
    const int rt = chain ? 1 : 0;
    auto row = [&](const char* name, const void* ptr, int cols, int ld, bool o, bool written) { add(name, ptr, N, cols, ld, o ? 0 : rt, written); };
    const bool enc = !oc;
    row("Xb", b.Xb, L.F + L.CTX, L.ld_xb, false, true);
    row("Hb1", b.Hb1, SP_H, SP_LDH, false, true); row("Hb2", b.Hb2, SP_H, SP_LDH, false, true);
    row("Ob", b.Ob, L.NP + 8, L.ld_ob, true, true);
    row("glimpse", b.glimpse, L.glimpse, L.ld_gl, false, true);
    row("He1", b.He1, SP_ENC_H1, SP_ENC_H1, false, enc); row("He2", b.He2, SP_ENC_H2, SP_ENC_H2, false, enc);
    row("Oe", b.Oe, 2 * L.A, L.ld_oe, true, true);
    row("Xz", b.Xz, L.x_depth, L.ld_x, false, true);
    row("Hz1", b.Hz1, SP_H, SP_LDH, false, true); row("Hz2", b.Hz2, SP_H, SP_LDH, false, true);
    row("Oz", b.Oz, L.NP + 2, L.ld_oz, true, true);
    row("Xo", b.Xo, L.x_depth + 1, L.ld_x, false, true);
    row("Ho1", b.Ho1, SP_H, SP_LDH, false, true); row("Ho2", b.Ho2, SP_H, SP_LDH, false, true);
    row("Oo", b.Oo, 1, L.ld_oo, true, true);
    row("dXb", b.dXb, L.F + L.CTX, L.ld_xb, false, !chain);
    row("dHb1", b.dHb1, SP_H, SP_LDH, false, true); row("dHb2", b.dHb2, SP_H, SP_LDH, false, true);
    row("dOb", b.dOb, L.NP + 8, L.ld_ob, false, true);
    add("dGl", b.dGl, N, L.glimpse, L.ld_gl, 0, !chain || input_grad);
    row("dHe1", b.dHe1, SP_ENC_H1, SP_ENC_H1, false, enc); row("dHe2", b.dHe2, SP_ENC_H2, SP_ENC_H2, false, enc);
    row("dOe", b.dOe, 2 * L.A, L.ld_oe, false, true);
    row("dXz", b.dXz, L.x_depth, L.ld_x, false, !chain);
    row("dHz1", b.dHz1, SP_H, SP_LDH, false, true); row("dHz2", b.dHz2, SP_H, SP_LDH, false, true);
    row("dOz", b.dOz, L.NP + 2, L.ld_oz, false, true);
    row("dXo", b.dXo, L.x_depth + 1, L.ld_x, false, !chain);
    row("dHo1", b.dHo1, SP_H, SP_LDH, false, true); row("dHo2", b.dHo2, SP_H, SP_LDH, false, true);
    row("dOo", b.dOo, 1, L.ld_oo, false, true);
    add("Za", w.Za, N, L.A, L.ld_rec, 0, !chain);
    add("Za16", w.Za16, N, L.A, L.ld_rec, 1, b16);
    const int per = d.P * d.P * (d.C + 1);
    add("Hd1", w.Hd1, N, SP_DEC_H1, SP_DEC_H1, et, !oc); add("Hd2", w.Hd2, N, SP_DEC_H2, SP_DEC_H2, et, !oc);
    add("dHd1", w.dHd1, N, SP_DEC_H1, SP_DEC_H1, et, !oc); add("dHd2", w.dHd2, N, SP_DEC_H2, SP_DEC_H2, et, !oc);
    add("S", w.S, N, per, w.ld_s, p.rp.s16 ? 2 : 0, true);
    add("dLog", w.dLog, N, per, w.ld_s, p.rp.g16 ? 1 : 0, true);
    add("dLog16", w.dLog16, N, per, w.ld_s, 1, true);
    const int Ip = d.I + d.pad_pre + d.pad_post, Ipw = d.Iw + d.pad_pre + d.pad_post_w;
    add("xpad", w.xpad, (long long)d.B * Ip * Ipw, d.C, d.C, 0, true);
    char nm[96];
    for (int i = 0; i < d.n_conv; ++i) {
        const ConvSpec& cs = PL.conv[i];
        const long long px = (long long)d.B * cs.hout * cs.wout;
        snprintf(nm, sizeof(nm), "act%d", i); add(nm, w.act[i], px, cs.cout, cs.cout, et, true);
        snprintf(nm, sizeof(nm), "dact%d", i); add(nm, w.dact[i], px, cs.cout, cs.cout, et, i > 0 || (p.stem_wgrad != STEM_PATCH && p.stem_wgrad != STEM_GEMM));
    }
    add("feat", w.feat, N, d.F, w.ld_feat, 0, true);
    add("dfeat", w.dfeat, N, d.F, w.ld_feat, 0, !chain);
    add("dfeat16", w.dfeat16, N, d.F, w.ld_feat, 1, true);
    for (int i = 1; i < PL.n_conv; ++i) {
        const ConvSpec& cs = PL.conv[i];
        const int K = cs.k * cs.k * cs.cin;
        snprintf(nm, sizeof(nm), "conv_wf%d", i); add(nm, w.conv_wf[i], cs.cout, K, round_up(K, 8), et, true);
        if (cs.k == 1) { snprintf(nm, sizeof(nm), "conv_wd%d_0", i); add(nm, w.conv_wd[i][0], cs.cin, cs.cout, round_up(cs.cout, 8), et, true); }
        else for (int q = 0; q < cs.s * cs.s; ++q) {
// ... 122 lines not shown
```

### spair_pytorch_amd/csrc/misc.h

```cpp
#pragma once
#include "common.h"

struct PrepEntry {
    const float* src;
    void* dst;
    int rows, cols, ld;
    int mode, bf16;
    int cin, cout, k, py, px, T, s;
    int KT, ksplit, kpad0, n_off;
};
#define SP_MAX_PREP 32
struct PrepTable {
    int n;
    PrepEntry e[SP_MAX_PREP];
};

int misc_pad_input(const float* x, float* xp, int B, int C, int I, int Iw, int pre, int Ip, int Ipw, hipStream_t s);
int misc_prep(const PrepTable& T, hipStream_t s);
int misc_export(const float* src, int ld, int col0, int ch, const int* cell_h, const int* cell_w, int B, int G, int Gw, float* out, hipStream_t s);
int misc_export16(const void* src, int ld, int col0, int ch, const int* cell_h, const int* cell_w, int B, int G, int Gw, float* out, hipStream_t s);
bool misc_conv0_reads_unpadded(int B, int Hin, int C, int k, int Cout);
bool misc_conv0_writes_mask(int B, int Hin, int C, int k, int s, int Cout, int out_bf16);
int misc_conv0_fwd(const float* x, const float* xp, const float* w, const float* bias, float* out, int B, int I, int pre, int Hin, int C, int k, int s,
                   int Hout, int Cout, int out_bf16, hipStream_t st, unsigned char* mask = nullptr, int Win = 0, int Wout = 0, bool unpadded = true);
int misc_conv0_wgrad(const float* xp, const float* dout, float* dw, int B, int Hin, int C, int k, int s, int Hout, int Cout, hipStream_t st);
```

### spair_pytorch_amd/csrc/misc.hip

```cpp
#include <cstdlib>
#include <cstring>
#include "cells.h"
#include "misc.h"

__global__ __launch_bounds__(256) void k_adam(float* __restrict__ p, const float* __restrict__ g, float* __restrict__ m,
                                              float* __restrict__ v, long long n, float lr, float b1, float b2, float eps,
                                              float bc1, float sqrt_bc2) {
    const long long i = (long long)blockIdx.x * blockDim.x + threadIdx.x;
    if (i >= n) return;
    const float gi = g[i];
    const float mi = b1 * m[i] + (1.f - b1) * gi;
    const float vi = b2 * v[i] + (1.f - b2) * gi * gi;
    m[i] = mi;
    v[i] = vi;
    const float denom = sqrtf(vi) / sqrt_bc2 + eps;
    p[i] -= (lr / bc1) * (mi / denom);
}

extern "C" int spair_adam(float* params, const float* grads, float* exp_avg, float* exp_avg_sq, int64_t n, float lr,
                          float beta1, float beta2, float eps, int step, void* stream) {
    if (n <= 0 || step < 1) return SPAIR_ERR_SHAPE;
    const float bc1 = 1.f - powf(beta1, (float)step);
    const float sqrt_bc2 = sqrtf(1.f - powf(beta2, (float)step));
    hipLaunchKernelGGL(k_adam, dim3((unsigned)((n + 255) / 256)), dim3(256), 0, (hipStream_t)stream, params, grads, exp_avg,
// ... 75 lines not shown

extern "C" int spair_noise_fill(const SpairDims* d, uint64_t seed, float* eps_box, float* eps_attr, float* eps_depth,
                                float* u_pres, void* stream) {
    if (!d) return SPAIR_ERR_SHAPE;
    const long long cells = (long long)d->B * d->G * (d->Gw ? d->Gw : d->G);
    const long long total = cells * (4 + d->A + 2);
    hipLaunchKernelGGL(k_noise, dim3((unsigned)((total + 255) / 256)), dim3(256), 0, (hipStream_t)stream, seed, eps_box, cells * 4,
                       eps_attr, cells * d->A, eps_depth, cells, u_pres, cells);
    SPAIR_CHECK_LAUNCH();
    return SPAIR_OK;
}

__global__ __launch_bounds__(256) void k_pad_input(const float* __restrict__ x, float* __restrict__ xp, int B, int C, int I, int Iw, int pre,
                                                   int Ip, int Ipw) {
    const long long idx = (long long)blockIdx.x * blockDim.x + threadIdx.x;
    const long long total = (long long)B * Ip * Ipw * C;
    if (idx >= total) return;
    const int c = (int)(idx % C);
    long long t = idx / C;
    const int px = (int)(t % Ipw); t /= Ipw;
    const int py = (int)(t % Ip);
    const int b = (int)(t / Ip);
    const int sx = px - pre, sy = py - pre;
    xp[idx] = (sx >= 0 && sx < Iw && sy >= 0 && sy < I) ? x[(((size_t)b * C + c) * I + sy) * Iw + sx] : 0.f;
}
int misc_pad_input(const float* x, float* xp, int B, int C, int I, int Iw, int pre, int Ip, int Ipw, hipStream_t s) {
    const long long total = (long long)B * Ip * Ipw * C;
    hipLaunchKernelGGL(k_pad_input, dim3((unsigned)((total + 255) / 256)), dim3(256), 0, s, x, xp, B, C, I, Iw, pre, Ip, Ipw);
    SPAIR_CHECK_LAUNCH();
    return SPAIR_OK;
}

__global__ __launch_bounds__(256) void k_prep(PrepTable T) {
    const PrepEntry e = T.e[blockIdx.y];
    if (e.mode == 4) {
        const int KP = e.KT * 32;
        const long long n4 = (long long)e.rows * KP;
        for (long long idx = (long long)blockIdx.x * blockDim.x + threadIdx.x; idx < n4; idx += (long long)gridDim.x * blockDim.x) {
            const int r = (int)(idx / KP), kk = (int)(idx - (long long)r * KP);
            int col = (kk < e.kpad0) ? (kk < e.ksplit ? kk : -1) : e.ksplit + (kk - e.kpad0);
            if (col >= e.cols) col = -1;
            float v = col >= 0 ? e.src[(size_t)r * e.cols + col] : 0.f;
            if (e.bf16 == 2) v -= (float)(__bf16)v;
            const int nn = e.n_off + r, nt = nn >> 4, li = nn & 15, kt = kk >> 5, g = (kk & 31) >> 3, j = kk & 7;
            reinterpret_cast<__bf16*>(e.dst)[(((size_t)nt * e.KT + kt) * 64 + g * 16 + li) * 8 + j] = (__bf16)v;
        }
        return;
    }
    if (e.mode == 5) {
        const long long n5 = (long long)e.rows * e.cols;
        for (long long idx = (long long)blockIdx.x * blockDim.x + threadIdx.x; idx < n5; idx += (long long)gridDim.x * blockDim.x) {
            const int o = (int)(idx / e.cols), i = (int)(idx - (long long)o * e.cols);
            const int kk = e.n_off + o, nt = i >> 4, li = i & 15, kt = kk >> 5, g = (kk & 31) >> 3, j = kk & 7;
            reinterpret_cast<__bf16*>(e.dst)[(((size_t)nt * e.KT + kt) * 64 + g * 16 + li) * 8 + j] = (__bf16)e.src[idx];
        }
        return;
    }
    const long long n = (long long)e.rows * e.cols;
    for (long long idx = (long long)blockIdx.x * blockDim.x + threadIdx.x; idx < n; idx += (long long)gridDim.x * blockDim.x) {
        const int r = (int)(idx / e.cols), c = (int)(idx - (long long)r * e.cols);
        float v;
        if (e.mode == 0) v = e.src[(size_t)r * e.cols + c];
        else if (e.mode == 1) v = e.src[(size_t)c * e.rows + r];
        else if (e.mode == 2) {
            int ky, kx, ci;
            if (e.s > 0) {
                const int blk = c >> 6, TT = e.T * e.T, nh = e.cin >> 6;
                const int tq = blk % TT, rr = blk / TT, h = rr % nh, cls = rr / nh;
                ky = cls / e.s + e.s * (tq / e.T); kx = cls % e.s + e.s * (tq % e.T); ci = h * 64 + (c & 63);
            } else {
                const int tap = c / e.cin;
                ci = c - tap * e.cin; ky = tap / e.k; kx = tap - ky * e.k;
            }
            v = e.src[(((size_t)r * e.cin + ci) * e.k + ky) * e.k + kx];
        } else {
            const int t = c / e.cout, co = c - t * e.cout, ty = t / e.T, tx = t - ty * e.T;
            v = e.src[(((size_t)co * e.cin + r) * e.k + (e.py + e.s * ty)) * e.k + (e.px + e.s * tx)];
        }
        const size_t o = (size_t)r * e.ld + c;
        if (e.bf16) reinterpret_cast<__bf16*>(e.dst)[o] = (__bf16)v;
        else reinterpret_cast<float*>(e.dst)[o] = v;
    }
}
int misc_prep(const PrepTable& T, hipStream_t s) {
    if (T.n <= 0) return SPAIR_OK;
    hipLaunchKernelGGL(k_prep, dim3(64, T.n), dim3(256), 0, s, T);
    SPAIR_CHECK_LAUNCH();
    return SPAIR_OK;
}

__global__ __launch_bounds__(256) void k_export(const float* __restrict__ src, int ld, int col0, int ch, const int* __restrict__ cell_h,
                                                const int* __restrict__ cell_w, int B, int G, int Gw, float* __restrict__ out) {
    const long long idx = (long long)blockIdx.x * blockDim.x + threadIdx.x;
    const long long total = (long long)B * G * Gw * ch;
    if (idx >= total) return;
    const int c = (int)(idx % ch);
    const long long r = idx / ch;
    const int cp = (int)(r / B), b = (int)(r - (long long)cp * B);
    out[(((size_t)b * ch + c) * G + cell_h[cp]) * Gw + cell_w[cp]] = src[r * ld + col0 + c];
}
__global__ __launch_bounds__(256) void k_export16(const __bf16* __restrict__ src, int ld, int col0, int ch, const int* __restrict__ cell_h,
                                                  const int* __restrict__ cell_w, int B, int G, int Gw, float* __restrict__ out) {
    const long long idx = (long long)blockIdx.x * blockDim.x + threadIdx.x;
    const long long total = (long long)B * G * Gw * ch;
    if (idx >= total) return;
    const int c = (int)(idx % ch);
    const long long r = idx / ch;
    const int cp = (int)(r / B), b = (int)(r - (long long)cp * B);
    out[(((size_t)b * ch + c) * G + cell_h[cp]) * Gw + cell_w[cp]] = (float)src[r * ld + col0 + c];
}
int misc_export16(const void* src, int ld, int col0, int ch, const int* cell_h, const int* cell_w, int B, int G, int Gw, float* out, hipStream_t s) {
    const long long total = (long long)B * G * Gw * ch;
    hipLaunchKernelGGL(k_export16, dim3((unsigned)((total + 255) / 256)), dim3(256), 0, s, reinterpret_cast<const __bf16*>(src), ld, col0, ch,
                       cell_h, cell_w, B, G, Gw, out);
    SPAIR_CHECK_LAUNCH();
    return SPAIR_OK;
}
int misc_export(const float* src, int ld, int col0, int ch, const int* cell_h, const int* cell_w, int B, int G, int Gw, float* out,
                hipStream_t s) {
    const long long total = (long long)B * G * Gw * ch;
    hipLaunchKernelGGL(k_export, dim3((unsigned)((total + 255) / 256)), dim3(256), 0, s, src, ld, col0, ch, cell_h, cell_w, B, G, Gw, out);
    SPAIR_CHECK_LAUNCH();
    return SPAIR_OK;
}

__global__ __launch_bounds__(256) void k_conv0_fwd(const float* __restrict__ xp, const float* __restrict__ w, const float* __restrict__ bias,
                                                   float* __restrict__ out, int B, int Hin, int Win, int C, int k, int s, int Hout, int Wout, int Cout,
                                                   int out_bf16) {
    extern __shared__ float wsh[];
    const int K0 = k * k * C;
    for (int i = threadIdx.x; i < K0 * Cout; i += blockDim.x) {
        const int co = i / K0, kk = i - co * K0;
        const int ci = kk / (k * k), rem = kk - ci * k * k;
        wsh[((rem * C) + ci) * Cout + co] = w[i];
    }
    __syncthreads();
    const int q = Cout / 4;
    const long long total = (long long)B * Hout * Wout * q;
    for (long long idx = (long long)blockIdx.x * blockDim.x + threadIdx.x; idx < total; idx += (long long)gridDim.x * blockDim.x) {
        const int cq = (int)(idx % q);
        const long long m = idx / q;
        const int ox = (int)(m % Wout), oy = (int)((m / Wout) % Hout), b = (int)(m / ((long long)Hout * Wout));
        float4 acc = *reinterpret_cast<const float4*>(bias + cq * 4);
        for (int ky = 0; ky < k; ++ky) {
            const float* row = xp + (((size_t)b * Hin + oy * s + ky) * Win + ox * s) * C;
            for (int t = 0; t < k * C; ++t) {
                const float xv = row[t];
                const float4 wv = *reinterpret_cast<const float4*>(&wsh[((ky * k * C) + t) * Cout + cq * 4]);
                acc.x += xv * wv.x; acc.y += xv * wv.y; acc.z += xv * wv.z; acc.w += xv * wv.w;
            }
        }
        acc.x = fmaxf(acc.x, 0.f); acc.y = fmaxf(acc.y, 0.f); acc.z = fmaxf(acc.z, 0.f); acc.w = fmaxf(acc.w, 0.f);
        if (out_bf16) {
            bf16x4 o;
            o[0] = (__bf16)acc.x; o[1] = (__bf16)acc.y; o[2] = (__bf16)acc.z; o[3] = (__bf16)acc.w;
            *reinterpret_cast<bf16x4*>(reinterpret_cast<__bf16*>(out) + (size_t)m * Cout + cq * 4) = o;
        } else {
            *reinterpret_cast<float4*>(out + (size_t)m * Cout + cq * 4) = acc;
        }
    }
}
constexpr int C0_ROWS = 5;
__global__ __launch_bounds__(256) void k_conv0_fwd_c1k4(const float* __restrict__ x, const float* __restrict__ w,
                                                        const float* __restrict__ bias, float* __restrict__ out, int Hin, int s,
                                                        int Hout, int Cout, int out_bf16, int I, int pre) {
    extern __shared__ float xs[];
    const int oy0 = blockIdx.x * C0_ROWS, b = blockIdx.y;
    const int nrow = min(C0_ROWS, Hout - oy0), nin = s * (nrow - 1) + 4;
    const int q = Cout >> 2, groups = 256 / q;
    const int cq = threadIdx.x % q, pg = threadIdx.x / q;
    {
        const __amdgpu_buffer_rsrc_t rsx = buf_rsrc(x + (size_t)b * I * I);
        const int total = nin * Hin;
        for (int i0 = threadIdx.x; i0 < total; i0 += 8 * 256) {
            unsigned v[8];
#pragma unroll
            for (int e = 0; e < 8; ++e) {
                const int i = i0 + e * 256;
                const int ky = i / Hin, xx = i - ky * Hin;
                const int sy = oy0 * s + ky - pre, sx = xx - pre;
                const bool in = i < total && (unsigned)sy < (unsigned)I && (unsigned)sx < (unsigned)I;
                v[e] = __builtin_amdgcn_raw_buffer_load_b32(rsx, in ? (sy * I + sx) * 4 : (int)BUF_OOB, 0, 0);
            }
#pragma unroll
            for (int e = 0; e < 8; ++e)
                if (i0 + e * 256 < total) xs[i0 + e * 256] = __uint_as_float(v[e]);
        }
    }
    typedef float f2 __attribute__((ext_vector_type(2)));
    f2 wlo[16], whi[16];
    {
        const float4* w4 = reinterpret_cast<const float4*>(w + (size_t)cq * 4 * 16);
        float4 t[16];
#pragma unroll
        for (int i = 0; i < 16; ++i) t[i] = w4[i];
#pragma unroll
        for (int tq = 0; tq < 4; ++tq) {
            wlo[tq * 4 + 0] = f2{t[tq].x, t[4 + tq].x}; whi[tq * 4 + 0] = f2{t[8 + tq].x, t[12 + tq].x};
            wlo[tq * 4 + 1] = f2{t[tq].y, t[4 + tq].y}; whi[tq * 4 + 1] = f2{t[8 + tq].y, t[12 + tq].y};
            wlo[tq * 4 + 2] = f2{t[tq].z, t[4 + tq].z}; whi[tq * 4 + 2] = f2{t[8 + tq].z, t[12 + tq].z};
            wlo[tq * 4 + 3] = f2{t[tq].w, t[4 + tq].w}; whi[tq * 4 + 3] = f2{t[8 + tq].w, t[12 + tq].w};
        }
    }
    const float4 bv = *reinterpret_cast<const float4*>(bias + cq * 4);
    __syncthreads();
    if (pg >= groups) return;
    const size_t mrow = ((size_t)b * Hout + oy0) * Hout;
    const int npix = nrow * Hout;
#pragma unroll 2
    for (int p = pg; p < npix; p += groups) {
        const int r = p / Hout, ox = p - r * Hout;
        const float* xr = xs + r * s * Hin + ox * s;
        f2 a0 = f2{bv.x, bv.y}, a1 = f2{bv.z, bv.w};
#pragma unroll
        for (int ky = 0; ky < 4; ++ky)
#pragma unroll
            for (int kx = 0; kx < 4; ++kx) {
                const float xv = xr[ky * Hin + kx];
                const f2 x2 = f2{xv, xv};
                a0 = __builtin_elementwise_fma(x2, wlo[ky * 4 + kx], a0);
                a1 = __builtin_elementwise_fma(x2, whi[ky * 4 + kx], a1);
            }
        float4 acc;
        acc.x = fmaxf(a0.x, 0.f); acc.y = fmaxf(a0.y, 0.f); acc.z = fmaxf(a1.x, 0.f); acc.w = fmaxf(a1.y, 0.f);
        if (out_bf16) {
            bf16x4 o;
            o[0] = (__bf16)acc.x; o[1] = (__bf16)acc.y; o[2] = (__bf16)acc.z; o[3] = (__bf16)acc.w;
            *reinterpret_cast<bf16x4*>(reinterpret_cast<__bf16*>(out) + (mrow + p) * Cout + cq * 4) = o;
        } else {
            *reinterpret_cast<float4*>(out + (mrow + p) * Cout + cq * 4) = acc;
        }
    }
}

typedef short c0_s16x4 __attribute__((ext_vector_type(4)));
constexpr int C0_TP = 272;
__device__ __forceinline__ void c0_split4(const float (&v)[4], c0_s16x4& hi, c0_s16x4& lo) {
    bf16x4 h, l;
#pragma unroll
    for (int e = 0; e < 4; ++e) {
        h[e] = (__bf16)v[e];
        l[e] = (__bf16)(v[e] - (float)h[e]);
    }
    hi = __builtin_bit_cast(c0_s16x4, h);
    lo = __builtin_bit_cast(c0_s16x4, l);
}
__host__ __device__ constexpr size_t c0_mfma_xs_bytes(int Hin) { return (((size_t)(2 * (C0_ROWS - 1) + 4) * (Hin + 2) * sizeof(float)) + 15) & ~(size_t)15; }
__global__ __launch_bounds__(256) void k_conv0_fwd_c1k4_mfma(const float* __restrict__ x, const float* __restrict__ w,
                                                             const float* __restrict__ bias, __bf16* __restrict__ out, int Hin, int Hout,
                                                             int I, int pre, unsigned char* __restrict__ mask) {
    extern __shared__ float xs[];
    char* tile = reinterpret_cast<char*>(xs) + c0_mfma_xs_bytes(Hin);
    const int oy0 = blockIdx.x * C0_ROWS, b = blockIdx.y;
    const int nrow = min(C0_ROWS, Hout - oy0), nin = 2 * (nrow - 1) + 4;
    const int tid = threadIdx.x, lane = tid & 63, wave = tid >> 6;
    const int LDX = Hin + 2;
    {
        const __amdgpu_buffer_rsrc_t rsx = buf_rsrc(x + (size_t)b * I * I);
        const int total = nin * LDX;
        for (int i0 = tid; i0 < total; i0 += 8 * 256) {
            unsigned v[8];
#pragma unroll
            for (int e = 0; e < 8; ++e) {
                const int i = i0 + e * 256;
                const int ky = i / LDX, xx = i - ky * LDX;
                const int sy = oy0 * 2 + ky - pre, sx = xx - pre;
                const bool in = i < total && (unsigned)sy < (unsigned)I && (unsigned)sx < (unsigned)I;
                v[e] = __builtin_amdgcn_raw_buffer_load_b32(rsx, in ? (sy * I + sx) * 4 : (int)BUF_OOB, 0, 0);
            }
#pragma unroll
            for (int e = 0; e < 8; ++e)
                if (i0 + e * 256 < total) xs[i0 + e * 256] = __uint_as_float(v[e]);
        }
    }
    const int q = lane >> 4, m = lane & 15;
    c0_s16x4 wh[8], wl[8];
    f32x4 bv[8];
#pragma unroll
    for (int g = 0; g < 8; ++g) {
        const int ch = 32 * (m >> 2) + 4 * g + (m & 3);
        const float4 t = *reinterpret_cast<const float4*>(w + (size_t)ch * 16 + q * 4);
        const float tv[4] = {t.x, t.y, t.z, t.w};
        c0_split4(tv, wh[g], wl[g]);
        const float4 bq = *reinterpret_cast<const float4*>(bias + 32 * q + 4 * g);
        bv[g] = (f32x4){bq.x, bq.y, bq.z, bq.w};
    }
    __syncthreads();
    const int nbx = (Hout + 15) >> 4, nblk = nrow * nbx;
    char* tw = tile + wave * (16 * C0_TP);
    for (int blk = wave; blk < nblk; blk += 4) {
        const int r = blk / nbx, ox0 = (blk - r * nbx) * 16;
        const int oxc = min(ox0 + m, Hout - 1);
        const float* xr = xs + (r * 2 + q) * LDX + oxc * 2;
        const float2 p0 = *reinterpret_cast<const float2*>(xr), p1 = *reinterpret_cast<const float2*>(xr + 2);
        const float pv[4] = {p0.x, p0.y, p1.x, p1.y};
        c0_s16x4 xh, xl;
        c0_split4(pv, xh, xl);
        f32x4 acc[8];
#pragma unroll
        for (int g = 0; g < 8; ++g) {
            acc[g] = __builtin_amdgcn_mfma_f32_16x16x16bf16_1k(wh[g], xh, bv[g], 0, 0, 0);
            acc[g] = __builtin_amdgcn_mfma_f32_16x16x16bf16_1k(wl[g], xh, acc[g], 0, 0, 0);
            acc[g] = __builtin_amdgcn_mfma_f32_16x16x16bf16_1k(wh[g], xl, acc[g], 0, 0, 0);
        }
#pragma unroll
        for (int j = 0; j < 4; ++j) {
            bf16x8 o;
#pragma unroll
            for (int e = 0; e < 4; ++e) {
                o[e] = (__bf16)fmaxf(acc[2 * j][e], 0.f);
                o[4 + e] = (__bf16)fmaxf(acc[2 * j + 1][e], 0.f);
            }
            *reinterpret_cast<bf16x8*>(tw + m * C0_TP + q * 64 + j * 16) = o;
        }
        wave_lds_fence();
        __bf16* drow = out + (((size_t)b * Hout + oy0 + r) * Hout + ox0) * 128;
        const int npx = min(16, Hout - ox0);
#pragma unroll
        for (int j = 0; j < 4; ++j) {
            const int px = 4 * j + q;
            const bf16x8 o = *reinterpret_cast<const bf16x8*>(tw + px * C0_TP + m * 16);
            if (px < npx) __builtin_nontemporal_store(o, reinterpret_cast<bf16x8*>(drow + px * 128 + m * 8));
            if (mask) {
                const u32x4_t wv = __builtin_bit_cast(u32x4_t, o);
                auto nz2 = [](unsigned v) { return (unsigned)((int)(v << 16) > 0) | ((unsigned)((int)v >> 16 > 0) << 1); };
                const unsigned byte = nz2(wv.x) | (nz2(wv.y) << 2) | (nz2(wv.z) << 4) | (nz2(wv.w) << 6);
                if (px < npx) mask[(((size_t)b * Hout + oy0 + r) * Hout + ox0 + px) * 16 + m] = (unsigned char)byte;
            }
        }
        wave_lds_fence();
    }
}

bool misc_conv0_reads_unpadded(int B, int Hin, int C, int k, int Cout) {
    return Cout % 4 == 0 && C == 1 && k == 4 && Cout / 4 <= 256 && 256 % (Cout / 4) == 0 && B <= 65535 &&
           (size_t)(4 * (C0_ROWS - 1) + 4) * Hin * sizeof(float) <= 48 * 1024;
}
bool misc_conv0_writes_mask(int B, int Hin, int C, int k, int s, int Cout, int out_bf16) {
    return misc_conv0_reads_unpadded(B, Hin, C, k, Cout) && out_bf16 && Cout == 128 && s == 2 && (Hin & 1) == 0;
}
int misc_conv0_fwd(const float* x, const float* xp, const float* w, const float* bias, float* out, int B, int I, int pre, int Hin, int C, int k,
                   int s, int Hout, int Cout, int out_bf16, hipStream_t st, unsigned char* mask, int Win, int Wout, bool unpadded) {
    if (Cout % 4) return SPAIR_ERR_ALIGN;
    if (Win == 0) { Win = Hin; Wout = Hout; }
    if (unpadded && Win == Hin && misc_conv0_reads_unpadded(B, Hin, C, k, Cout)) {
        if (s < 1 || s > 4) return SPAIR_ERR_UNSUPPORTED;
        if (out_bf16 && Cout == 128 && s == 2 && (Hin & 1) == 0) {
            hipLaunchKernelGGL(k_conv0_fwd_c1k4_mfma, dim3((Hout + C0_ROWS - 1) / C0_ROWS, B), dim3(256), c0_mfma_xs_bytes(Hin) + 4 * 16 * C0_TP, st, x,
                               w, bias, reinterpret_cast<__bf16*>(out), Hin, Hout, I, pre, mask);
            SPAIR_CHECK_LAUNCH();
            return SPAIR_OK;
        }
        hipLaunchKernelGGL(k_conv0_fwd_c1k4, dim3((Hout + C0_ROWS - 1) / C0_ROWS, B), dim3(256),
                           (size_t)(s * (C0_ROWS - 1) + 4) * Hin * sizeof(float), st, x, w, bias, out, Hin, s, Hout, Cout, out_bf16, I, pre);
        SPAIR_CHECK_LAUNCH();
        return SPAIR_OK;
    }
    const size_t lds = (size_t)k * k * C * Cout * sizeof(float);
    if (lds > 64 * 1024) return SPAIR_ERR_UNSUPPORTED;
    const long long total = (long long)B * Hout * Wout * (Cout / 4);
    const unsigned grid = (unsigned)min((long long)4096, (total + 255) / 256);
    hipLaunchKernelGGL(k_conv0_fwd, dim3(grid), dim3(256), lds, st, xp, w, bias, out, B, Hin, Win, C, k, s, Hout, Wout, Cout, out_bf16);
    SPAIR_CHECK_LAUNCH();
    return SPAIR_OK;
}

extern "C" int spair_stem_conv_fwd(const float* x, const float* w, const float* bias, void* out, int B, int I, int pad_pre, int Hin, int Hout,
                                   int Cout, int stride, int out_bf16, void* stream) {
    if (!x || !w || !bias || !out) return SPAIR_ERR_SHAPE;
    if (B <= 0 || I <= 0 || stride < 1 || Hin < I + pad_pre || Hout != (Hin - 4) / stride + 1) return SPAIR_ERR_SHAPE;
    if (!misc_conv0_reads_unpadded(B, Hin, 1, 4, Cout)) return SPAIR_ERR_UNSUPPORTED;
    return misc_conv0_fwd(x, nullptr, w, bias, reinterpret_cast<float*>(out), B, I, pad_pre, Hin, 1, 4, stride, Hout, Cout, out_bf16, (hipStream_t)stream);
}
extern "C" int spair_stem_conv_fwd_mask(const float* x, const float* w, const float* bias, void* out, void* mask8, int B, int I, int pad_pre, int Hin,
                                        int Hout, void* stream) {
    if (!x || !w || !bias || !out || !mask8) return SPAIR_ERR_SHAPE;
    if (B <= 0 || I <= 0 || Hin < I + pad_pre || Hout != (Hin - 4) / 2 + 1) return SPAIR_ERR_SHAPE;
    if (!misc_conv0_writes_mask(B, Hin, 1, 4, 2, 128, 1)) return SPAIR_ERR_UNSUPPORTED;
    return misc_conv0_fwd(x, nullptr, w, bias, reinterpret_cast<float*>(out), B, I, pad_pre, Hin, 1, 4, 2, Hout, 128, 1, (hipStream_t)stream,
                          reinterpret_cast<unsigned char*>(mask8));
}

__global__ __launch_bounds__(256) void k_conv0_wgrad(const float* __restrict__ xp, const float* __restrict__ dout, float* __restrict__ dw,
                                                     int B, int Hin, int C, int k, int s, int Hout, int Cout, int rows_per_block) {
    extern __shared__ float sh[];
    const int K0 = k * k * C;
    float* dsh = sh;
    float* psh = sh + 64 * Cout;
    const long long M = (long long)B * Hout * Hout;
    const long long m_beg = (long long)blockIdx.x * rows_per_block, m_end = min(M, m_beg + rows_per_block);
    const int npair = Cout * K0;
    float acc[8] = {0.f, 0.f, 0.f, 0.f, 0.f, 0.f, 0.f, 0.f};
    for (long long m0 = m_beg; m0 < m_end; m0 += 64) {
        const int nr = (int)min((long long)64, m_end - m0);
        __syncthreads();
        for (int i = threadIdx.x; i < nr * Cout; i += blockDim.x) dsh[i] = dout[(size_t)m0 * Cout + i];
        for (int i = threadIdx.x; i < nr * K0; i += blockDim.x) {
            const int rr = i / K0, kk = i - rr * K0;
            const long long m = m0 + rr;
            const int ox = (int)(m % Hout), oy = (int)((m / Hout) % Hout), b = (int)(m / ((long long)Hout * Hout));
            const int tap = kk / C, ci = kk - tap * C, ky = tap / k, kx = tap - ky * k;
            psh[i] = xp[(((size_t)b * Hin + oy * s + ky) * Hin + ox * s + kx) * C + ci];
        }
        __syncthreads();
#pragma unroll
        for (int i = 0; i < 8; ++i) {
            const int p = threadIdx.x + i * 256;
            if (p >= npair) break;
            const int co = p % Cout, kk = p / Cout;
// ... 27 lines not shown
```

Before: 84310.

## Fuse stem conv0 into conv1 patch kernel and split weight prep for overlap

Adds a STEM variant of the conv1 s2k4 patch kernel. It computes the conv0 stem (split-bf16 MFMA) on the fly from the raw input and writes that output straight into the LDS patch buffer, while still storing act0 and its relu bits for backward. This removes the separate stem kernel launch and the round trip of act0 through memory before conv1 reads it. Weight prep is also split: conv1 forward weights are prepped first on more workgroups, and the remaining weights go to a second pass behind a new event that conv2 waits on, so that prep overlaps conv1. In exchange the loader waves carry more register pressure and a more complex pipeline, and the stem work is redone per patch tile.

```diff
diff --git a/include/spair_hip.h b/include/spair_hip.h
--- a/include/spair_hip.h
+++ b/include/spair_hip.h
@@ -102,6 +102,7 @@
 #define SPAIR_STEM_WGRAD16 2
 #define SPAIR_STEM_GENERIC 3
 int spair_step_plan(const SpairDims* d, const void* workspace, int flags, int input_grad, int* out, int n);
+int spair_step_plan_stem_fwd(const SpairDims* d, const void* workspace, int flags, int input_grad);
 int spair_workspace_view(const SpairDims* d, const void* workspace, int flags, int input_grad, const char* name, long long* out);
 int spair_workspace_view_name(const SpairDims* d, int idx, char* name, int name_cap);
 int spair_chain_stamp_wavefronts(const SpairDims* d);
@@ -176,6 +177,10 @@
                             void* out16, int B, int Ho, void* stream);
 int spair_stem_conv_fwd_mask(const float* x, const float* w, const float* bias, void* out, void* mask8, int B, int I, int pad_pre, int Hin,
                              int Hout, void* stream);
+int spair_conv_s2k4_fwd16_mask(const void* in16, const void* wf16, const float* bias, void* out16, void* mask8, int B, int Hin, int Hout,
+                               void* stream);
+int spair_conv1_stem_fwd16(const float* x, const float* w0, const float* b0, void* act0, void* bits0, const void* wf16, const float* bias,
+                           void* out16, void* mask8, int B, int I, int pad_pre, int Hin, int Hout, void* stream);
 int spair_conv_s2k4_dgrad16_bits(const void* dout16, const void* wd0, const void* wd1, const void* wd2, const void* wd3,
                                  const void* gate_bits8, void* out16, int B, int Ho, void* stream);
 int64_t spair_decoder_fwd16_scratch_bytes(int n_out);
diff --git a/spair_pytorch_amd/_lib.py b/spair_pytorch_amd/_lib.py
--- a/spair_pytorch_amd/_lib.py
+++ b/spair_pytorch_amd/_lib.py
@@ -66,6 +66,8 @@
                                              ctypes.POINTER(ctypes.c_int), ctypes.c_int])):
             f.argtypes, f.restype = args, ctypes.c_int
         _declare_parse(h)
+        h.spair_step_plan_stem_fwd.argtypes = [ctypes.POINTER(SpairDims), ctypes.c_void_p, ctypes.c_int, ctypes.c_int]
+        h.spair_step_plan_stem_fwd.restype = ctypes.c_int
         _lib = h
     return _lib
 
@@ -119,6 +121,26 @@
                 dgrad=tuple(CONV_KERNELS[out[22 + i]] for i in layers), gate_bits=tuple(bool(out[30 + i]) for i in layers))
 
 
+def step_plan_stem_fwd(dims, workspace, flags=0, input_grad=False):
+    rc = lib().spair_step_plan_stem_fwd(ctypes.byref(dims), ctypes.c_void_p(int(workspace)), int(flags), int(bool(input_grad)))
+    if rc < 0:
+        check(rc, "spair_step_plan_stem_fwd")
+    return bool(rc)
+
+
+def conv1_stem_fwd16(x, w0, b0, wf16, bias, act0, bits0, out16, mask8, pad_pre):
+    B, I = int(x.shape[0]), int(x.shape[1])
+    Hin, Hout = int(act0.shape[1]), int(out16.shape[1])
+    for t in (x, w0, b0, wf16, bias, act0, bits0, out16, mask8):
+        if not t.is_contiguous():
+            raise SpairHipError("conv1_stem_fwd16: operands must be contiguous")
+    if x.shape != (B, I, I) or act0.shape != (B, Hin, Hin, 128) or bits0.shape != (B, Hin, Hin, 16) or out16.shape != (B, Hout, Hout, 128) or \
+            mask8.shape != (B, Hout, Hout, 16) or w0.numel() != 128 * 16 or b0.numel() != 128 or wf16.shape != (128, 2048) or bias.numel() != 128:
+        raise SpairHipError("conv1_stem_fwd16: bad operand shapes")
+    check(lib().spair_conv1_stem_fwd16(ptr(x), ptr(w0), ptr(b0), ptr(act0), ptr(bits0), ptr(wf16), ptr(bias), ptr(out16), ptr(mask8),
+                                       B, I, int(pad_pre), Hin, Hout, stream()), "spair_conv1_stem_fwd16")
+
+
 VIEW_DTYPES = (torch.float32, torch.bfloat16, torch.float16)
 
 
diff --git a/spair_pytorch_amd/csrc/backbone.h b/spair_pytorch_amd/csrc/backbone.h
--- a/spair_pytorch_amd/csrc/backbone.h
+++ b/spair_pytorch_amd/csrc/backbone.h
@@ -5,6 +5,9 @@
 bool conv_s2k4_patch_fwd16_supported(int B, int Hin, int Hout, int cin, int cout, int k, int s_);
 int conv_s2k4_patch_fwd16(const void* in, const void* wf, const float* bias, void* out, int B, int Hin, int Hout, int cin, int cout, int k, int s_,
                           hipStream_t s, void* mask = nullptr);
+bool conv_s2k4_patch_stem_fwd16_supported(int B, int I, int pre, int Hin, int Hout);
+int conv_s2k4_patch_stem_fwd16(const float* x, const float* w0, const float* b0, void* act0, void* bits0, const void* wf, const float* bias, void* out,
+                               void* mask, int B, int I, int pre, int Hin, int Hout, hipStream_t s);
 bool conv_s2k4_patch_dgrad16_supported(int B, int Ho, int hin, int cin, int cout, int k, int s_);
 bool conv_s2k4_patch_dgrad16_stem_supported(int B, int Ho, int hin, int cin, int cout, int k, int s_, int stem_hin, int stem_s, long long stem_part_cap);
 int conv_s2k4_patch_dgrad16(const void* dout, const void* const* wd, const void* gate, void* out, int B, int Ho, int hin, int cin, int cout, int k,
diff --git a/spair_pytorch_amd/csrc/chain.hip b/spair_pytorch_amd/csrc/chain.hip
--- a/spair_pytorch_amd/csrc/chain.hip
+++ b/spair_pytorch_amd/csrc/chain.hip
@@ -164,9 +164,6 @@
 }
 __device__ __forceinline__ void buf_store8_nt(__amdgpu_buffer_rsrc_t r, unsigned byte_off, unsigned lo, unsigned hi) {
     __builtin_amdgcn_raw_buffer_store_b64(u32x2_t{lo, hi}, r, (int)byte_off, 0, 2);
-}
-__device__ __forceinline__ void buf_store16_nt(__amdgpu_buffer_rsrc_t r, unsigned byte_off, u32x4_t v) {
-    __builtin_amdgcn_raw_buffer_store_b128(v, r, (int)byte_off, 0, 2);
 }
 
 template <int KT>
diff --git a/spair_pytorch_amd/csrc/common.h b/spair_pytorch_amd/csrc/common.h
--- a/spair_pytorch_amd/csrc/common.h
+++ b/spair_pytorch_amd/csrc/common.h
@@ -112,6 +112,24 @@
 __device__ __forceinline__ void buf_store16(__amdgpu_buffer_rsrc_t r, unsigned byte_off, uint4 v) {
     __builtin_amdgcn_raw_buffer_store_b128(u32x4_t{v.x, v.y, v.z, v.w}, r, (int)byte_off, 0, 0);
 }
+__device__ __forceinline__ void buf_store16_nt(__amdgpu_buffer_rsrc_t r, unsigned byte_off, u32x4_t v) {
+    __builtin_amdgcn_raw_buffer_store_b128(v, r, (int)byte_off, 0, 2);
+}
+__device__ __forceinline__ unsigned relu_bits2(unsigned w) { return (unsigned)((int)(w << 16) > 0) | ((unsigned)((int)w >> 16 > 0) << 1); }
+__device__ __forceinline__ unsigned relu_bits8(unsigned x, unsigned y, unsigned z, unsigned w) {
+    return relu_bits2(x) | (relu_bits2(y) << 2) | (relu_bits2(z) << 4) | (relu_bits2(w) << 6);
+}
+typedef short c0_s16x4 __attribute__((ext_vector_type(4)));
+__device__ __forceinline__ void c0_split4(const float (&v)[4], c0_s16x4& hi, c0_s16x4& lo) {
+    bf16x4 h, l;
+#pragma unroll
+    for (int e = 0; e < 4; ++e) {
+        h[e] = (__bf16)v[e];
+        l[e] = (__bf16)(v[e] - (float)h[e]);
+    }
+    hi = __builtin_bit_cast(c0_s16x4, h);
+    lo = __builtin_bit_cast(c0_s16x4, l);
+}
 #endif
 
 __device__ __forceinline__ float block_reduce_sum_256(float v, float* smem4) {
diff --git a/spair_pytorch_amd/csrc/conv_s2.hip b/spair_pytorch_amd/csrc/conv_s2.hip
--- a/spair_pytorch_amd/csrc/conv_s2.hip
+++ b/spair_pytorch_amd/csrc/conv_s2.hip
@@ -22,7 +22,22 @@
 template <int W>
 __device__ __forceinline__ void cp_wait() { asm volatile("s_waitcnt vmcnt(%0)" ::"n"(W) : "memory"); }
 
-__global__ __launch_bounds__(768, 3) void k_conv_s2k4_patch(ConvPatchArgs a) {
+struct ConvStemArgs {
+    const float* x; const float* w0; const float* b0;
+    unsigned char* bits0;
+    int I, pre;
+};
+constexpr int CS_NBLK = 2;
+constexpr int CS_PRO = 4;
+
+#define CS_WAIT_TAPS(T, N)                                                                                                                   \
+    asm volatile("s_waitcnt vmcnt(%8)"                                                                                                       \
+                 : "+v"(T[0][0]), "+v"(T[0][1]), "+v"(T[0][2]), "+v"(T[0][3]), "+v"(T[1][0]), "+v"(T[1][1]), "+v"(T[1][2]), "+v"(T[1][3])    \
+                 : "n"(N)                                                                                                                    \
+                 : "memory")
+
+template <bool STEM>
+__device__ __forceinline__ void cp_body(const ConvPatchArgs& a, const ConvStemArgs& sa) {
     extern __shared__ __attribute__((aligned(16))) char cp_sm[];
     char* bt = cp_sm;
     char* patch = cp_sm + 3 * CP_BT_B;
@@ -74,31 +89,166 @@
         }
     };
 
+    int E0 = 0, x0 = 0, bb0 = 0, y0 = 0, nown = 0;
+    float rWs = 0.f, rHs = 0.f;
+    u32x4_t rx_s = {0, 0, 0, 0};
+    __amdgpu_buffer_rsrc_t ract0 = rin, rbits0 = rin;
+    c0_s16x4 wh[2][4], wl[2][4];
+    f32x4 bv[2][4];
+    if constexpr (STEM) {
+        E0 = L0 / Ws; x0 = L0 - E0 * Ws; bb0 = E0 / Hs; y0 = E0 - bb0 * Hs;
+        rWs = 1.f / (float)Ws; rHs = 1.f / (float)Hs;
+        const int gm = mend / Hout;
+        nown = mend < a.M ? (gm + gm / Hout) * Ws + (mend - gm * Hout) - L0 : npx;
+        const unsigned long long xa = reinterpret_cast<unsigned long long>(sa.x);
+        rx_s = u32x4_t{(unsigned)__builtin_amdgcn_readfirstlane((unsigned)xa), (unsigned)__builtin_amdgcn_readfirstlane((unsigned)(xa >> 32)),
+                       0xffffff00u, 0x00020000u};
+        ract0 = buf_rsrc(a.in); rbits0 = buf_rsrc(sa.bits0);
+    }
+    auto stem_weights = [&](int h, const float* w0, const float* b0) {
+#pragma unroll
+        for (int g = 0; g < 4; ++g) {
+            const int ch = h * 64 + 16 * (r16 >> 2) + 4 * g + (r16 & 3);
+            const float4 t = *reinterpret_cast<const float4*>(w0 + (size_t)ch * 16 + q * 4);
+            const float tv[4] = {t.x, t.y, t.z, t.w};
+            c0_split4(tv, wh[h][g], wl[h][g]);
+            const float4 bq = *reinterpret_cast<const float4*>(b0 + h * 64 + 16 * q + 4 * g);
+            bv[h][g] = (f32x4){bq.x, bq.y, bq.z, bq.w};
+        }
+    };
+    auto stem_issue = [&](int sn, int blk, unsigned (&v)[4], int& pix) {
+        const int cls = sn >> 1, py = cls >> 1, px = cls & 1;
+        int pp = blk * 16 + r16;
+        asm volatile("" : "+v"(pp));
+        const int n1 = x0 + pp, q1 = (int)(((float)n1 + 0.5f) * rWs), xx = n1 - q1 * Ws;
+        const int n2 = y0 + q1, q2 = (int)(((float)n2 + 0.5f) * rHs), yy = n2 - q2 * Hs, b = bb0 + q2;
+        const bool ok = sn < 8 && pp < npx && b < a.B;
+        const int Y = 2 * yy + py, X = 2 * xx + px;
+        const int sy = 2 * Y - sa.pre + q, sx = 2 * X - sa.pre;
+        const bool rok = ok && (unsigned)sy < (unsigned)sa.I;
+        const int ro = (b * sa.I + sy) * sa.I + sx;
+#pragma unroll
+        for (int e = 0; e < 4; ++e) {
+            const unsigned off = rok && (unsigned)(sx + e) < (unsigned)sa.I ? (unsigned)(ro + e) * 4u : BUF_OOB;
+            asm volatile("buffer_load_dword %0, %1, %2, 0 offen" : "=v"(v[e]) : "v"(off), "s"(rx_s) : "memory");
+        }
+        pix = ok && pp < nown ? (b * a.Hin + Y) * a.Hin + X : -1;
+    };
+    auto stem_block = [&](int h, bool live, int blk, const unsigned (&v)[4], int pix, char* dst) {
+        u32x4_t o0 = {0u, 0u, 0u, 0u}, o1 = o0;
+        if (live) {
+            const float pv[4] = {__uint_as_float(v[0]), __uint_as_float(v[1]), __uint_as_float(v[2]), __uint_as_float(v[3])};
+            c0_s16x4 xh, xl;
+            c0_split4(pv, xh, xl);
+            f32x4 sacc[4];
+#pragma unroll
+            for (int g = 0; g < 4; ++g) {
+                sacc[g] = __builtin_amdgcn_mfma_f32_16x16x16bf16_1k(wh[h][g], xh, bv[h][g], 0, 0, 0);
+                sacc[g] = __builtin_amdgcn_mfma_f32_16x16x16bf16_1k(wl[h][g], xh, sacc[g], 0, 0, 0);
+                sacc[g] = __builtin_amdgcn_mfma_f32_16x16x16bf16_1k(wh[h][g], xl, sacc[g], 0, 0, 0);
+            }
+            bf16x8 t0, t1;
+#pragma unroll
+            for (int e = 0; e < 4; ++e) {
+                t0[e] = (__bf16)fmaxf(sacc[0][e], 0.f); t0[4 + e] = (__bf16)fmaxf(sacc[1][e], 0.f);
+                t1[e] = (__bf16)fmaxf(sacc[2][e], 0.f); t1[4 + e] = (__bf16)fmaxf(sacc[3][e], 0.f);
+            }
+            o0 = __builtin_bit_cast(u32x4_t, t0); o1 = __builtin_bit_cast(u32x4_t, t1);
+            int pp = blk * 16 + r16;
+            asm volatile("" : "+v"(pp));
+            char* row = pp < CP_PPX ? dst + pp * 128 : cp_sm + 3 * CP_BT_B + 2 * CP_PATCH_B + (pp - CP_PPX) * 128;
+            const unsigned l0 = (unsigned)(size_t)(__attribute__((address_space(3))) char*)(row + (((2 * q) ^ (pp & 7)) << 4));
+            const unsigned l1 = (unsigned)(size_t)(__attribute__((address_space(3))) char*)(row + (((2 * q + 1) ^ (pp & 7)) << 4));
+            asm volatile("ds_write_b128 %0, %1" ::"v"(l0), "v"(o0) : "memory");
+            asm volatile("ds_write_b128 %0, %1" ::"v"(l1), "v"(o1) : "memory");
+        }
+        const unsigned ao = pix >= 0 ? (unsigned)pix * 256u + (unsigned)(h * 128 + q * 32) : BUF_OOB;
+        buf_store16_nt(ract0, ao, o0);
+        buf_store16_nt(ract0, pix >= 0 ? ao + 16u : BUF_OOB, o1);
+        const unsigned bits = relu_bits8(o0.x, o0.y, o0.z, o0.w) | (relu_bits8(o1.x, o1.y, o1.z, o1.w) << 8);
+        buf_store2(rbits0, pix >= 0 ? (unsigned)pix * 16u + (unsigned)(h * 8 + 2 * q) : BUF_OOB, (unsigned short)bits);
+    };
+
     f32x4 acc[4][4];
-#pragma unroll
-    for (int i = 0; i < 4; ++i)
-#pragma unroll
-        for (int j = 0; j < 4; ++j) acc[i][j] = (f32x4){0.f, 0.f, 0.f, 0.f};
-
     if (loader) {
-#pragma unroll
-        for (int part = 0; part < 3; ++part) issue_patch(0, part);
-        issue_b(0);
-        issue_b(1);
-        cp_wait<4>();
-        for (int st = 0; st < 8; ++st) {
-#pragma unroll
-            for (int j4 = 0; j4 < 4; ++j4) {
-                const int kt = st * 4 + j4;
-                __builtin_amdgcn_s_barrier();
-                asm volatile("" ::: "memory");
-                if (j4 != 3) issue_patch(st + 1, j4);
-                issue_b(kt + 2);
-                if (j4 == 3) cp_wait<4>(); else cp_wait<4 + CP_NPIECE_W>();
-            }
-        }
-        __builtin_amdgcn_s_barrier();
+        if constexpr (STEM) {
+            const float *w0l = sa.w0, *b0l = sa.b0;
+            asm volatile("" : "+s"(w0l), "+s"(b0l));
+            stem_weights(0, w0l, b0l);
+            stem_weights(1, w0l, b0l);
+            unsigned lv[2][CS_NBLK][4];
+            int lpix[2][CS_NBLK];
+            issue_b(0);
+            issue_b(1);
+#pragma unroll
+            for (int e = 0; e < CS_NBLK; ++e) stem_issue(1, lw * CS_NBLK + e, lv[0][e], lpix[0][e]);
+            cp_wait<4 + 4 * CS_NBLK>();
+            for (int c2 = 0; c2 < 4; ++c2) {
+#pragma unroll
+                for (int h = 0; h < 2; ++h) {
+                    const int st = c2 * 2 + h;
+                    char* dst = patch + (1 - h) * CP_PATCH_B;
+#pragma unroll
+                    for (int j4 = 0; j4 < 4; ++j4) {
+                        const int kt = st * 4 + j4, cur = j4 & 1, nxt = cur ^ 1;
+                        __builtin_amdgcn_s_barrier();
+                        asm volatile("" ::: "memory");
+                        issue_b(kt + 2);
+#pragma unroll
+                        for (int e = 0; e < CS_NBLK; ++e)
+                            stem_issue(((kt + 1) >> 2) + 1, (((kt + 1) & 3) * 4 + lw) * CS_NBLK + e, lv[nxt][e], lpix[nxt][e]);
+                        if (h == 0 && j4 == 0 && c2 == 0) CS_WAIT_TAPS(lv[cur], 4 + 4 * CS_NBLK);
+                        else CS_WAIT_TAPS(lv[cur], 4 + 4 * CS_NBLK + 3 * CS_NBLK);
+#pragma unroll
+                        for (int e = 0; e < CS_NBLK; ++e) {
+                            const int blk = (j4 * 4 + lw) * CS_NBLK + e;
+                            stem_block(1 - h, st < 7 && blk * 16 < npx, blk, lv[cur][e], lpix[cur][e], dst);
+                        }
+                        asm volatile("s_waitcnt lgkmcnt(0)" ::: "memory");
+                    }
+                }
+            }
+            __builtin_amdgcn_s_barrier();
+        } else {
+#pragma unroll
+            for (int part = 0; part < 3; ++part) issue_patch(0, part);
+            issue_b(0);
+            issue_b(1);
+            cp_wait<4>();
+            for (int st = 0; st < 8; ++st) {
+#pragma unroll
+                for (int j4 = 0; j4 < 4; ++j4) {
+                    const int kt = st * 4 + j4;
+                    __builtin_amdgcn_s_barrier();
+                    asm volatile("" ::: "memory");
+                    if (j4 != 3) issue_patch(st + 1, j4);
+                    issue_b(kt + 2);
+                    if (j4 == 3) cp_wait<4>(); else cp_wait<4 + CP_NPIECE_W>();
+                }
+            }
+            __builtin_amdgcn_s_barrier();
+        }
     } else {
+        if constexpr (STEM) {
+            stem_weights(0, sa.w0, sa.b0);
+            unsigned pv[CS_PRO][4];
+            int ppix[CS_PRO];
+#pragma unroll
+            for (int i = 0; i < CS_PRO; ++i) stem_issue(0, wave + 8 * i, pv[i], ppix[i]);
+            asm volatile("s_waitcnt vmcnt(0)"
+                         : "+v"(pv[0][0]), "+v"(pv[0][1]), "+v"(pv[0][2]), "+v"(pv[0][3]), "+v"(pv[1][0]), "+v"(pv[1][1]), "+v"(pv[1][2]),
+                           "+v"(pv[1][3]), "+v"(pv[2][0]), "+v"(pv[2][1]), "+v"(pv[2][2]), "+v"(pv[2][3]), "+v"(pv[3][0]), "+v"(pv[3][1]),
+                           "+v"(pv[3][2]), "+v"(pv[3][3])
+                         :
+                         : "memory");
+#pragma unroll
+            for (int i = 0; i < CS_PRO; ++i) stem_block(0, (wave + 8 * i) * 16 < npx, wave + 8 * i, pv[i], ppix[i], patch);
+            asm volatile("s_waitcnt lgkmcnt(0)" ::: "memory");
+        }
+#pragma unroll
+        for (int i = 0; i < 4; ++i)
+#pragma unroll
+            for (int j = 0; j < 4; ++j) acc[i][j] = (f32x4){0.f, 0.f, 0.f, 0.f};
         int pbase[4];
 #pragma unroll
         for (int i = 0; i < 4; ++i) {
@@ -162,13 +312,15 @@
             const uint4 v = *reinterpret_cast<const uint4*>(cs + row * CP_LDC + ch);
             buf_store16(rout, (m0 + row) < mend ? ((unsigned)(m0 + row) * CP_C + ch) * 2u : BUF_OOB, v);
             if (a.mask) {
-                auto nz2 = [](unsigned w) { return (unsigned)((int)(w << 16) > 0) | ((unsigned)((int)w >> 16 > 0) << 1); };
-                const unsigned byte = nz2(v.x) | (nz2(v.y) << 2) | (nz2(v.z) << 4) | (nz2(v.w) << 6);
+                const unsigned byte = relu_bits8(v.x, v.y, v.z, v.w);
                 if ((m0 + row) < mend) a.mask[(size_t)(m0 + row) * 16 + (tid & 15)] = (unsigned char)byte;
             }
         }
     }
 }
+
+__global__ __launch_bounds__(768, 3) void k_conv_s2k4_patch(ConvPatchArgs a) { cp_body<false>(a, ConvStemArgs{}); }
+__global__ __launch_bounds__(768, 3) void k_conv_s2k4_patch_stem(ConvPatchArgs a, ConvStemArgs sa) { cp_body<true>(a, sa); }
 
 }
 
@@ -217,6 +369,44 @@
     return SPAIR_OK;
 }
 
+static int cs_plan(int B, int I, int pre, int Hin, int Hout, int& tiles, int& tpi) {
+    const int rc = cp_plan(B, Hin, Hout, CP_C, CP_C, 4, 2, tiles, tpi);
+    if (rc != SPAIR_OK) return rc;
+    if (I <= 0 || pre < 0 || I + pre > 2 * Hin + 2 || (long long)B * I * I >= (1ll << 30) || Hout + 1 + 16 * 36 >= 2048) return SPAIR_ERR_UNSUPPORTED;
+    return SPAIR_OK;
+}
+bool conv_s2k4_patch_stem_fwd16_supported(int B, int I, int pre, int Hin, int Hout) {
+    int t, p;
+    return cs_plan(B, I, pre, Hin, Hout, t, p) == SPAIR_OK;
+}
+int conv_s2k4_patch_stem_fwd16(const float* x, const float* w0, const float* b0, void* act0, void* bits0, const void* wf, const float* bias, void* out,
+                               void* mask, int B, int I, int pre, int Hin, int Hout, hipStream_t s) {
+    int tiles = 0, tpi = 0;
+    { const int rc = cs_plan(B, I, pre, Hin, Hout, tiles, tpi); if (rc != SPAIR_OK) return rc; }
+    static std::atomic<unsigned long long> attr_done{0};
+    if (spair_dyn_lds_once(reinterpret_cast<const void*>(&k_conv_s2k4_patch_stem), CP_LDS, attr_done) != SPAIR_OK) return SPAIR_ERR_LAUNCH;
+    ConvPatchArgs a;
+    a.in = reinterpret_cast<const u16*>(act0); a.wf = reinterpret_cast<const u16*>(wf); a.bias = bias; a.out = reinterpret_cast<u16*>(out);
+    a.mask = reinterpret_cast<unsigned char*>(mask);
+    a.B = B; a.Hin = Hin; a.Hout = Hout; a.M = B * Hout * Hout; a.K = 16 * CP_C; a.tpi = tpi;
+    ConvStemArgs sa;
+    sa.x = x; sa.w0 = w0; sa.b0 = b0; sa.bits0 = reinterpret_cast<unsigned char*>(bits0); sa.I = I; sa.pre = pre;
+    hipLaunchKernelGGL(k_conv_s2k4_patch_stem, dim3(tiles), dim3(768), CP_LDS, s, a, sa);
+    SPAIR_CHECK_LAUNCH();
+    return SPAIR_OK;
+}
+
+extern "C" int spair_conv1_stem_fwd16(const float* x, const float* w0, const float* b0, void* act0, void* bits0, const void* wf16, const float* bias,
+                                      void* out16, void* mask16, int B, int I, int pad_pre, int Hin, int Hout, void* stream) {
+    if (!x || !w0 || !b0 || !act0 || !bits0 || !wf16 || !bias || !out16 || !mask16) return SPAIR_ERR_SHAPE;
+    return conv_s2k4_patch_stem_fwd16(x, w0, b0, act0, bits0, wf16, bias, out16, mask16, B, I, pad_pre, Hin, Hout, (hipStream_t)stream);
+}
+
 extern "C" int spair_conv_s2k4_fwd16(const void* in16, const void* wf16, const float* bias, void* out16, int B, int Hin, int Hout, void* stream) {
     return conv_s2k4_patch_fwd16(in16, wf16, bias, out16, B, Hin, Hout, 128, 128, 4, 2, (hipStream_t)stream);
 }
+extern "C" int spair_conv_s2k4_fwd16_mask(const void* in16, const void* wf16, const float* bias, void* out16, void* mask8, int B, int Hin, int Hout,
+                                          void* stream) {
+    if (!mask8) return SPAIR_ERR_SHAPE;
+    return conv_s2k4_patch_fwd16(in16, wf16, bias, out16, B, Hin, Hout, 128, 128, 4, 2, (hipStream_t)stream, mask8);
+}
diff --git a/spair_pytorch_amd/csrc/engine.hip b/spair_pytorch_amd/csrc/engine.hip
--- a/spair_pytorch_amd/csrc/engine.hip
+++ b/spair_pytorch_amd/csrc/engine.hip
@@ -129,6 +129,7 @@
     bool stem_bits;
     StemWgrad stem_wgrad;
     bool stem_unpadded;
+    bool conv1_stem;
     bool dec_dgrad_fused;
     bool dec_wgrad_grouped;
     bool dec_wgrad_late;
@@ -193,6 +194,8 @@
         } else p.conv_dgrad[i] = CONV_PER_CLASS;
         bits = p.conv_fwd[i] == CONV_PATCH;
     }
+    p.conv1_stem = b16 && grey4 && !(flags & 128) && p.stem_bits && p.stem_unpadded && n > 1 && p.conv_fwd[1] == CONV_PATCH &&
+                   PL.conv[1].hin == c0.hout && conv_s2k4_patch_stem_fwd16_supported(d.B, d.I, d.pad_pre, PL.conv[1].hin, PL.conv[1].hout);
     const bool dec16 = b16 && !PL.oc_n;
     p.dec_dgrad_fused = dec16 && !(flags & 64) && dec_fused_bwd_supported(PL.lin[LIN_DEC0].in, per, L.N, ld_s, ld_s, L.ld_rec);
     p.dec_wgrad_grouped = dec16 && decoder_small_wgrad_grouped_supported(PL, L);
@@ -580,17 +583,20 @@
         e.cin = cin; e.cout = cout; e.k = k; e.py = py; e.px = px; e.T = T; e.s = s;
         es.push_back(e);
     };
-    for (int i = 1; part == 0 && i < c.PL.n_conv; ++i) {
+    for (int i = 1; part != 1 && i < c.PL.n_conv; ++i) {
         const ConvSpec& cs = c.PL.conv[i];
         const float* w = c.params + cs.w;
         const int K = cs.k * cs.k * cs.cin;
+        const bool first = part == 0;
+        if (first && i > 1) break;
         if (cs.k == 1) {
-            push(w, c.w.conv_wf[i], cs.cout, cs.cin, round_up(K, 8), 0, bf);
-            if (need_dgrad) push(w, c.w.conv_wd[i][0], cs.cin, cs.cout, round_up(cs.cout, 8), 1, bf);
+            if (first == (i == 1)) push(w, c.w.conv_wf[i], cs.cout, cs.cin, round_up(K, 8), 0, bf);
+            if (need_dgrad && !first) push(w, c.w.conv_wd[i][0], cs.cin, cs.cout, round_up(cs.cout, 8), 1, bf);
         } else {
             const bool perm = conv_kperm(c, cs);
-            push(w, c.w.conv_wf[i], cs.cout, K, round_up(K, 8), 2, bf, cs.cin, cs.cout, cs.k, 0, 0, perm ? cs.k / cs.s : 0, perm ? cs.s : 0);
-            if (need_dgrad) {
+            if (first == (i == 1))
+                push(w, c.w.conv_wf[i], cs.cout, K, round_up(K, 8), 2, bf, cs.cin, cs.cout, cs.k, 0, 0, perm ? cs.k / cs.s : 0, perm ? cs.s : 0);
+            if (need_dgrad && !first) {
                 const int T = cs.k / cs.s;
                 for (int py = 0; py < cs.s; ++py)
                     for (int px = 0; px < cs.s; ++px)
@@ -647,7 +653,7 @@
         PrepTable T;
         T.n = (int)std::min((size_t)SP_MAX_PREP, es.size() - i);
         for (int j = 0; j < T.n; ++j) T.e[j] = es[i + j];
-        TRY(misc_prep(T, c.s));
+        TRY(misc_prep(T, c.s, part == 0 ? 256 : 64));
     }
     return SPAIR_OK;
 }
@@ -716,12 +722,15 @@
     return misc_conv0_fwd(c.x, c.w.xpad, c.params + c0.w, c.params + c0.b, c.w.act[0], d.B, d.I, d.pad_pre, c0.hin, d.C, c0.k, c0.s, c0.hout,
                           c0.cout, b16, c.s, c.w.act0_bits, c0.win, c0.wout, c.stem_unpadded);
 }
-static int backbone_fwd(Ctx& c) {
+static int backbone_fwd(Ctx& c, hipEvent_t rest_ready) {
     const SpairDims& d = c.d;
     const int b16 = d.dtype == SPAIR_BF16;
     const int pw0 = c.pw0;
+    const ConvSpec& c0 = c.PL.conv[0];
     for (int i = 1; i < c.PL.n_conv; ++i) {
         const ConvSpec& cs = c.PL.conv[i];
+        if ((i == 2 || (i == 1 && c.conv_fwd[1] == CONV_PW_STACK)) && rest_ready && hipStreamWaitEvent(c.s, rest_ready, 0) != hipSuccess)
+            return SPAIR_ERR_LAUNCH;
         const bool last = (i == c.PL.n_conv - 1);
         const int M = d.B * cs.hout * cs.wout, K = cs.k * cs.k * cs.cin;
         if (c.conv_fwd[i] == CONV_PW_STACK) {
@@ -737,7 +746,11 @@
         float* out = last ? c.w.feat : c.w.act[i];
         const int ldc = last ? c.w.ld_feat : cs.cout;
         const ConvDesc cd = fwd_desc(cs);
-        if (c.conv_fwd[i] == CONV_PATCH) {
+        if (i == 1 && c.conv1_stem) {
+            ProfScope ps(PS_CONV1_FWD, c.s);
+            TRY(conv_s2k4_patch_stem_fwd16(c.x, c.params + c0.w, c.params + c0.b, c.w.act[0], c.w.act0_bits, c.w.conv_wf[1], c.params + cs.b, out,
+                                           c.w.act_bits[1], d.B, d.I, d.pad_pre, cs.hin, cs.hout, c.s));
+        } else if (c.conv_fwd[i] == CONV_PATCH) {
             ProfScope ps(i == 1 ? PS_CONV1_FWD : -1, c.s);
             TRY(conv_s2k4_patch_fwd16(c.w.act[i - 1], c.w.conv_wf[i], c.params + cs.b, out, d.B, cs.hin, cs.hout, cs.cin, cs.cout, cs.k, cs.s, c.s,
                                       c.w.act_bits[i]));
@@ -1052,6 +1065,8 @@
             ProfScope ps(PS_PREP, c.s);
             TRY(prep_weights(c, st->train != 0, 0));
             if (side && hipEventRecord(side->ev[3], side->s) != hipSuccess) return SPAIR_ERR_LAUNCH;
+            TRY(prep_weights(c, st->train != 0, 2));
+            if (side && hipEventRecord(side->ev[5], side->s) != hipSuccess) return SPAIR_ERR_LAUNCH;
             TRY(cells_init_tables(d->G, d->Gw, c.L.LB, c.w.cell_h, c.w.cell_w, c.w.cidx, c.w.nbr, c.w.cons, c.w.diag_start, c.s));
             if (st->draw_noise)
                 TRY(spair_noise_fill(d, st->noise_seed, io->eps_box, io->eps_attr, io->eps_depth, io->u_pres, c.s));
@@ -1061,9 +1076,9 @@
         if (c.stem_unpadded) TRY(misc_pad_input(c.x, c.w.xpad, d->B, d->C, d->I, d->Iw, d->pad_pre, c.PL.conv[0].hin, c.PL.conv[0].win, c.s));
     }
     const int ps_bb = prof_begin(PS_BACKBONE_FWD, c.s);
-    TRY(backbone_stem_fwd(c));
+    if (!c.conv1_stem) TRY(backbone_stem_fwd(c));
     if (side && hipStreamWaitEvent(c.s, side->ev[3], 0) != hipSuccess) return SPAIR_ERR_LAUNCH;
-    TRY(backbone_fwd(c));
+    TRY(backbone_fwd(c, side ? side->ev[5] : nullptr));
     prof_end(ps_bb, c.s);
     if (side && hipStreamWaitEvent(c.s, side->ev[4], 0) != hipSuccess) return SPAIR_ERR_LAUNCH;
     { ProfScope ps(PS_CELLS_FWD, c.s); TRY(cells_fwd(c)); }
@@ -1453,6 +1468,13 @@
     }
     for (int i = 0; i < std::min(n, SPAIR_STEP_PLAN_INTS); ++i) out[i] = v[i];
     return SPAIR_OK;
+}
+
+extern "C" int spair_step_plan_stem_fwd(const SpairDims* d0, const void* workspace, int flags, int input_grad) {
+    if (!d0 || !workspace) return SPAIR_ERR_SHAPE;
+    const SpairDims dn = spair_dims_norm(*d0);
+    TRY(validate(dn));
+    return plan_step(dn, flags, input_grad != 0, workspace).conv1_stem ? 1 : 0;
 }
 
 struct WsItem { char name[96]; const void* p; long long rows, cols, ld; int type, written; };
diff --git a/spair_pytorch_amd/csrc/misc.h b/spair_pytorch_amd/csrc/misc.h
--- a/spair_pytorch_amd/csrc/misc.h
+++ b/spair_pytorch_amd/csrc/misc.h
@@ -16,7 +16,7 @@
 };
 
 int misc_pad_input(const float* x, float* xp, int B, int C, int I, int Iw, int pre, int Ip, int Ipw, hipStream_t s);
-int misc_prep(const PrepTable& T, hipStream_t s);
+int misc_prep(const PrepTable& T, hipStream_t s, int wgs_per_entry = 64);
 int misc_export(const float* src, int ld, int col0, int ch, const int* cell_h, const int* cell_w, int B, int G, int Gw, float* out, hipStream_t s);
 int misc_export16(const void* src, int ld, int col0, int ch, const int* cell_h, const int* cell_w, int B, int G, int Gw, float* out, hipStream_t s);
 bool misc_conv0_reads_unpadded(int B, int Hin, int C, int k, int Cout);
diff --git a/spair_pytorch_amd/csrc/misc.hip b/spair_pytorch_amd/csrc/misc.hip
--- a/spair_pytorch_amd/csrc/misc.hip
+++ b/spair_pytorch_amd/csrc/misc.hip
@@ -181,9 +181,9 @@
         else reinterpret_cast<float*>(e.dst)[o] = v;
     }
 }
-int misc_prep(const PrepTable& T, hipStream_t s) {
+int misc_prep(const PrepTable& T, hipStream_t s, int wgs_per_entry) {
     if (T.n <= 0) return SPAIR_OK;
-    hipLaunchKernelGGL(k_prep, dim3(64, T.n), dim3(256), 0, s, T);
+    hipLaunchKernelGGL(k_prep, dim3(wgs_per_entry, T.n), dim3(256), 0, s, T);
     SPAIR_CHECK_LAUNCH();
     return SPAIR_OK;
 }
@@ -332,18 +332,7 @@
     }
 }
 
-typedef short c0_s16x4 __attribute__((ext_vector_type(4)));
 constexpr int C0_TP = 272;
-__device__ __forceinline__ void c0_split4(const float (&v)[4], c0_s16x4& hi, c0_s16x4& lo) {
-    bf16x4 h, l;
-#pragma unroll
-    for (int e = 0; e < 4; ++e) {
-        h[e] = (__bf16)v[e];
-        l[e] = (__bf16)(v[e] - (float)h[e]);
-    }
-    hi = __builtin_bit_cast(c0_s16x4, h);
-    lo = __builtin_bit_cast(c0_s16x4, l);
-}
 __host__ __device__ constexpr size_t c0_mfma_xs_bytes(int Hin) { return (((size_t)(2 * (C0_ROWS - 1) + 4) * (Hin + 2) * sizeof(float)) + 15) & ~(size_t)15; }
 __global__ __launch_bounds__(256) void k_conv0_fwd_c1k4_mfma(const float* __restrict__ x, const float* __restrict__ w,
                                                              const float* __restrict__ bias, __bf16* __restrict__ out, int Hin, int Hout,
@@ -422,8 +411,7 @@
             if (px < npx) __builtin_nontemporal_store(o, reinterpret_cast<bf16x8*>(drow + px * 128 + m * 8));
             if (mask) {
                 const u32x4_t wv = __builtin_bit_cast(u32x4_t, o);
-                auto nz2 = [](unsigned v) { return (unsigned)((int)(v << 16) > 0) | ((unsigned)((int)v >> 16 > 0) << 1); };
-                const unsigned byte = nz2(wv.x) | (nz2(wv.y) << 2) | (nz2(wv.z) << 4) | (nz2(wv.w) << 6);
+                const unsigned byte = relu_bits8(wv.x, wv.y, wv.z, wv.w);
                 if (px < npx) mask[(((size_t)b * Hout + oy0 + r) * Hout + ox0 + px) * 16 + m] = (unsigned char)byte;
             }
         }
```

Result: slower. 82420 (-2.2%).
